# crstnbr/detqmc

Measured on AMD Instinct MI355X. Metric: DQMC sweeps/sec (SDW-O2 L=16 beta=10 fp64), higher is better.
Workload: dtype f64; 1 GPU; DetSDW O(2) L=16 beta=10 dtau=0.1 s=10 checkerboard delayed(32) sweepThermalization, 512 independent chains per GPU (1 process x 4 kernel contexts x 128 lockstep chains), stabilisation=qr; n_g=512, m=100, replicas_per_gpu=512, processes_per_gpu=1, contexts_per_process=4, chains_per_context=128, launch=self

## Files before the change

detqmc_amd/_lib.py:

```python
import ctypes as C
import os

HERE = os.path.dirname(os.path.abspath(__file__))
LIB_PATH = os.path.join(HERE, "lib", "libdetqmc_amd.so")


class DqmcError(RuntimeError):

    def __init__(self, code, msg):
        super().__init__(f"[dqmc {code}] {msg}")
        self.code = code


DQMC_TD_EVERY_SLICE = 0x100
DETSDW_TD_EVERY_SLICE = 0x100
DETSDW_TD_FINE_ON_DEVICE = 0x200
DETSDW_OBS_FINE = 0x100
DQMC_SERIES_AUTO_REBIN, DQMC_SERIES_TRACK_VARIANCE = 1, 2
DETSDW_SERIES_NO_HOST_COPY = 1
DETSDW_SERIES_PHI = 2
DETSDW_FM_EQ_CORRELATORS = 0x100
DQMC_TD_PH_BAND = 0x100
DETSDW_TD_PH_BAND = 0x100
DETSDW_FM_EQ_BAND = 0x200
DQMC_SERIES_MATS_BAND, DQMC_SERIES_EQ_BAND = 128, 256
DQMC_SERIES_MATS_CUSTOM, DQMC_SERIES_EQ_CUSTOM = 512, 1024
DQMC_SERIES_MATS_CUSTOM_PAIR, DQMC_SERIES_EQ_CUSTOM_PAIR = 2048, 4096
DQMC_SERIES_GREEN_MATRIX = 8192
DQMC_CUSTOM_MAX = 4
DETSDW_OBS_FAMILY_SLICE, DETSDW_OBS_FAMILY_EQ, DETSDW_OBS_FAMILY_TD, DETSDW_OBS_FAMILY_PHI = 0, 1, 2, 3
(DETSDW_OBS_KIND_SITE, DETSDW_OBS_KIND_TAU, DETSDW_OBS_KIND_TAU_Q0, DETSDW_OBS_KIND_ROW_SCALAR, DETSDW_OBS_KIND_CORR, DETSDW_OBS_KIND_SQ,
 DETSDW_OBS_KIND_GREEN_MATRIX, DETSDW_OBS_KIND_PHI_CHI, DETSDW_OBS_KIND_PHI_SCALARS) = range(9)


class dqmc_cplx(C.Structure):
    _fields_ = [("re", C.c_double), ("im", C.c_double)]


class dqmc_tuning(C.Structure):
    _fields_ = [("pipeline", C.c_int32), ("qr_variant", C.c_int32), ("green_variant", C.c_int32),
                ("max_jacobi_sweeps", C.c_int32), ("proposal_budget", C.c_int32), ("decide_threads", C.c_int32), ("bmult_path", C.c_int32)]


DQMC_TUNING_NO_RNG_LOOKAHEAD = 0x100


class dqmc_schedule_info(C.Structure):
    _fields_ = [("pipelined", C.c_int32), ("proposal_budget", C.c_int32), ("blocks_pipelined", C.c_uint64),
                ("blocks_sequential", C.c_uint64), ("qr_block_gram_schmidt", C.c_int32), ("green_lu", C.c_int32),
                ("cholqr_fallbacks", C.c_uint64), ("uniform_windows_advanced", C.c_uint64), ("uniform_windows_pushed", C.c_uint64)]


class dqmc_params(C.Structure):
    _fields_ = [("opdim", C.c_int32), ("L", C.c_int32), ("m", C.c_int32), ("s", C.c_int32),
                ("delaySteps", C.c_int32), ("bc", C.c_int32), ("weakZflux", C.c_int32),
                ("phi2bosons", C.c_int32), ("device", C.c_int32), ("stabilisation", C.c_int32),
                ("cb_none", C.c_int32), ("model", C.c_int32),
                ("dtau", C.c_double), ("r", C.c_double), ("c", C.c_double), ("u", C.c_double),
                ("lambda_", C.c_double),
                ("txhor", C.c_double), ("txver", C.c_double), ("tyhor", C.c_double), ("tyver", C.c_double),
                ("mux", C.c_double), ("muy", C.c_double), ("accRatio", C.c_double), ("cdwU", C.c_double),
                ("rng_window_per_site", C.c_int32), ("timedisplaced", C.c_int32),
                ("tuning", dqmc_tuning), ("td_particle_hole", C.c_int32)]


class dqmc_update_state(C.Structure):
    _fields_ = [("phiDelta", C.c_double), ("targetAccRatio", C.c_double), ("lastAccRatio", C.c_double),
                ("ra_runningAverage", C.c_double), ("ra_values", C.c_double * 100),
                ("ra_samplesAdded", C.c_int32), ("ra_head", C.c_int32),
                ("rng_consumed", C.c_uint64), ("rng_avail", C.c_uint64),
                ("error", C.c_int32), ("reserved", C.c_int32),
                ("angleDelta", C.c_double), ("scaleDelta", C.c_double),
                ("curminAngleDelta", C.c_double), ("curmaxAngleDelta", C.c_double),
                ("curminScaleDelta", C.c_double), ("curmaxScaleDelta", C.c_double),
                ("rot_runningAverage", C.c_double), ("rot_values", C.c_double * 100),
                ("scl_runningAverage", C.c_double), ("scl_values", C.c_double * 100),
                ("rot_samplesAdded", C.c_int32), ("rot_head", C.c_int32), ("scl_samplesAdded", C.c_int32), ("scl_head", C.c_int32)]


class dqmc_series_state(C.Structure):
    _fields_ = [("bin_size", C.c_int), ("max_bins", C.c_int), ("nfreq", C.c_int), ("parts", C.c_int), ("flags", C.c_int),
                ("bins_closed", C.c_int), ("sweeps_in_open_bin", C.c_int), ("nb", C.c_int),
                ("samples", C.c_longlong), ("rebins", C.c_longlong), ("sample_len", C.c_size_t)]


class dqmc_profile(C.Structure):
    _fields_ = [("ms", C.c_double * 8), ("launches", C.c_uint64 * 8),
                ("svd_calls", C.c_uint64), ("svd_sweeps_total", C.c_uint64), ("svd_sweeps_max", C.c_uint64),
                ("qr_calls", C.c_uint64), ("gemm_flops", C.c_double), ("decomp_round_ms", C.c_double),
                ("decomp_rounds", C.c_uint64), ("blocks_nonempty", C.c_uint64), ("chains", C.c_uint64),
                ("updates_accepted", C.c_uint64), ("lu_calls", C.c_uint64),
                ("sub_ms", C.c_double * 4), ("sub_launches", C.c_uint64 * 4), ("sub_flops", C.c_double * 4), ("sub_bytes", C.c_double * 4)]


class detsdw_params(C.Structure):
    _fields_ = [("opdim", C.c_int32), ("L", C.c_int32), ("m", C.c_int32), ("s", C.c_int32),
                ("delaySteps", C.c_int32), ("globalShift", C.c_int32), ("globalUpdateInterval", C.c_int32),
                ("weakZflux", C.c_int32), ("phi2bosons", C.c_int32), ("device", C.c_int32),
                ("simindex", C.c_int32), ("rngSeed", C.c_uint32), ("has_mux_muy", C.c_int32),
                ("updateMethod", C.c_int32), ("bc", C.c_char * 16),
                ("beta", C.c_double), ("dtau", C.c_double),
                ("r", C.c_double), ("c", C.c_double), ("u", C.c_double), ("lambda_", C.c_double),
                ("txhor", C.c_double), ("txver", C.c_double), ("tyhor", C.c_double), ("tyver", C.c_double),
                ("mu", C.c_double), ("mux", C.c_double), ("muy", C.c_double),
                ("accRatio", C.c_double), ("cdwU", C.c_double),
                ("stabilisation", C.c_int32), ("cb_none", C.c_int32),
                ("wolffClusterUpdate", C.c_int32), ("wolffClusterShiftUpdate", C.c_int32),
                ("repeatWolffPerSweep", C.c_int32), ("fermionMeasurements", C.c_int32),
                ("spinProposalMethod", C.c_int32), ("adaptScaleVariance", C.c_int32), ("repeatUpdateInSlice", C.c_int32),
                ("timeDisplacedMeasurements", C.c_int32),
                ("tuning", dqmc_tuning), ("timeDisplacedParticleHole", C.c_int32)]


class detsdw_info(C.Structure):
    _fields_ = [("opdim", C.c_int32), ("L", C.c_int32), ("N", C.c_int32), ("MSF", C.c_int32),
                ("n_g", C.c_int32), ("m", C.c_int32), ("s", C.c_int32), ("n", C.c_int32),
                ("performedSweeps", C.c_int32), ("lastSweepDir", C.c_int32),
                ("acceptedGlobalShifts", C.c_int32), ("attemptedGlobalShifts", C.c_int32),
                ("currentTimeslice", C.c_int32), ("reserved", C.c_int32),
                ("acceptedWolffClusterUpdates", C.c_int32), ("attemptedWolffClusterUpdates", C.c_int32),
                ("acceptedWolffClusterShiftUpdates", C.c_int32), ("attemptedWolffClusterShiftUpdates", C.c_int32),
                ("addedWolffClusterSize", C.c_double),
                ("beta", C.c_double), ("dtau", C.c_double),
                ("phiDelta", C.c_double), ("lastAccRatioLocal_phi", C.c_double), ("r", C.c_double),
                ("angleDelta", C.c_double), ("scaleDelta", C.c_double),
                ("rngDrawn", C.c_uint64)]


class detsdw_observable_desc(C.Structure):
    _fields_ = [(f, C.c_int32) for f in ("family", "block", "component", "kind", "fine", "has_fine_twin", "has_matsubara",
                                          "series_part", "series_bit")]


# ... 306 lines not shown
```

detqmc_amd/csrc/dqmc_context.hip:

```cpp
#include "dqmc_ctx.h"
#include <cmath>
#include <complex>
#include <cstddef>
#include <cstdio>
#include <cstdlib>
#include <cstring>
#include <string>
#include <vector>

void build_tournament(int nblk, std::vector<int>& out);

thread_local std::string g_err;

template<class T>
static int dalloc(dqmc_ctx* c, T** p, size_t count) {
    const size_t bytes = (count * sizeof(T) + 255) & ~(size_t)255;
    *p = (T*)(uintptr_t)(c->arena_off + 256);
    c->fixups.push_back((void**)p);
    c->arena_off += bytes;
    return 0;
}
static int arena_commit(dqmc_ctx* c) {
    const size_t cs = c->arena_off;
    void* q = nullptr;
// ... 229 lines not shown
    const double t = p.txhor, mu = p.mux;
    std::vector<hc> Em, Ep;
    if (p.cb_none) {
        std::vector<hc> T((size_t)N * N, hc(0.0));
        for (int i = 0; i < N; ++i) T[(size_t)i * N + i] = -mu;
        for (int site = 0; site < N; ++site)
            for (int dir = 0; dir < 4; ++dir) T[(size_t)neigh[dir * N + site] * N + site] -= t;
        herm_exp_dense(N, T, -p.dtau, +p.dtau, Em, Ep);
    } else {
        const double ch = std::cosh(p.dtau * t), sh = std::sinh(p.dtau * t);
        auto bond_matrix = [&](int dirn, int parity, double shv) {
            std::vector<double> M((size_t)N * N, 0.0);
            for (int i = 0; i < N; ++i) M[(size_t)i * N + i] = ch;
            for (int y = 0; y < L; ++y)
                for (int x = 0; x < L; ++x) {
                    const int coord = dirn == 0 ? x : y;
                    if ((coord & 1) != parity) continue;
                    const int a = y * L + x, b = neigh[(dirn == 0 ? 0 : 2) * N + a];
                    M[(size_t)a * N + b] += shv; M[(size_t)b * N + a] += shv;
                }
            return M;
        };
        auto mul = [&](const std::vector<double>& A, const std::vector<double>& B) {
            std::vector<double> C((size_t)N * N, 0.0);
            for (int i = 0; i < N; ++i) for (int k = 0; k < N; ++k) { const double a = A[(size_t)i * N + k]; if (a != 0.0) for (int j = 0; j < N; ++j) C[(size_t)i * N + j] += a * B[(size_t)k * N + j]; }
            return C;
        };
        const std::vector<double> F = mul(mul(bond_matrix(0, 0, sh), bond_matrix(0, 1, sh)), mul(bond_matrix(1, 0, sh), bond_matrix(1, 1, sh)));
        const std::vector<double> Fi = mul(mul(bond_matrix(1, 1, -sh), bond_matrix(1, 0, -sh)), mul(bond_matrix(0, 1, -sh), bond_matrix(0, 0, -sh)));
        Em.assign((size_t)N * N, hc(0.0)); Ep.assign((size_t)N * N, hc(0.0));
        for (size_t i = 0; i < (size_t)N * N; ++i) { Em[i] = F[i]; Ep[i] = Fi[i]; }
    }
    out_minus.assign((size_t)ng * ng, hc(0.0)); out_plus.assign((size_t)ng * ng, hc(0.0));
    for (int b = 0; b < 2; ++b)
        for (int i = 0; i < N; ++i) for (int j = 0; j < N; ++j) {
            out_minus[(size_t)(b * N + j) * ng + (b * N + i)] = Em[(size_t)i * N + j];
            out_plus[(size_t)(b * N + j) * ng + (b * N + i)] = Ep[(size_t)i * N + j];
        }
}

static int alloc_qr_work(dqmc_ctx* c) {
    const int ng = c->n_g, np = (ng + 15) / 16;
    const size_t n2 = (size_t)ng * ng;
    int rc;
#define A_(x) if ((rc = (x))) return rc;
    A_(dalloc(c, &c->qw.V, n2)); A_(dalloc(c, &c->qw.T, (size_t)np * 2 * 256));
    A_(dalloc(c, &c->qw.W, (size_t)16 * ng)); A_(dalloc(c, &c->qw.W2, (size_t)16 * ng)); A_(dalloc(c, &c->qw.Rneg, (size_t)32 * ng));
    if (ng > 1024) { c->qw.part_count = (size_t)ng * 64 * 8; A_(dalloc(c, &c->qw.part, c->qw.part_count)); }
    A_(dalloc(c, &c->qr_perm, (size_t)ng)); A_(dalloc(c, &c->lu_swaps, (size_t)LU_SWAP_INTS)); A_(dalloc(c, &c->lu_tneg, (size_t)ng * 32)); A_(dalloc(c, &c->qr_perm_inv, (size_t)ng)); A_(dalloc(c, &c->qr_dinv, (size_t)ng));
    A_(dalloc(c, &c->rmax_inv, (size_t)ng)); A_(dalloc(c, &c->rmin, (size_t)ng));
    A_(dalloc(c, &c->lmax_inv, (size_t)ng)); A_(dalloc(c, &c->lmin, (size_t)ng));
#undef A_
    return 0;
}

static int alloc_slot(dqmc_ctx* c, UdVSlot& sl) {
    size_t n2 = (size_t)c->n_g * c->n_g;
    int rc;
    if ((rc = dalloc(c, &sl.U, n2))) return rc;
    if ((rc = dalloc(c, &sl.d, (size_t)c->n_g))) return rc;
    if ((rc = dalloc(c, &sl.Vt, n2))) return rc;
    return 0;
}

extern "C" int dqmc_create(const dqmc_params* p, dqmc_ctx** out) { return dqmc_create_batch(p, 1, out); }
static int create_fill(dqmc_ctx* c, const dqmc_params* p);

extern "C" int dqmc_create_batch(const dqmc_params* p, int nchains, dqmc_ctx** out) {
    if (!p || !out) return fail(DQMC_EINVAL, "null argument");
    *out = nullptr;
    if (nchains < 1 || nchains > 1024) return fail(DQMC_EINVAL, "nchains must be in 1..1024");
    if (p->opdim < 1 || p->opdim > 3) return fail(DQMC_EINVAL, "opdim must be 1, 2 or 3");
    if (p->L < 2 || (p->L % 2) != 0)
        return fail(DQMC_EINVAL, "Checker board decomposition only supported for even linear lattice sizes");
    if (p->weakZflux && p->opdim != 2) return fail(DQMC_EINVAL, "Magnetic field currently only supported for opdim=2");
    if (p->m < 2 || p->s < 1 || p->s >= p->m) return fail(DQMC_EINVAL, "need 0 < s < m");
    const int N = p->L * p->L, MSF = p->opdim == 3 ? 4 : 2;
    if (p->delaySteps < 1 || p->delaySteps > N) return fail(DQMC_EINVAL, "delaySteps must be in 1..N");
    if (MSF * p->delaySteps > DQMC_MAX_WDIM) return fail(DQMC_EINVAL, "MSF*delaySteps must be <= 64 on this build");
    if (p->bc < 0 || p->bc > 3) return fail(DQMC_EINVAL, "bc");
    if (p->tuning.decide_threads != 0 && p->tuning.decide_threads != 256 && p->tuning.decide_threads != 512)
        return fail(DQMC_EINVAL, "tuning.decide_threads must be 0, 256 or 512");
    {
        const int path = p->tuning.bmult_path & ~DQMC_TUNING_NO_RNG_LOOKAHEAD;
        if (p->tuning.bmult_path < 0 || path > 2) return fail(DQMC_EINVAL, "tuning.bmult_path must be 0, 1 or 2");
    }
    if (p->stabilisation != DQMC_STAB_SVD && p->stabilisation != DQMC_STAB_QR) return fail(DQMC_EINVAL, "stabilisation");
    if (!(p->dtau > 0)) return fail(DQMC_EINVAL, "dtau");
    if (p->model != DQMC_MODEL_SDW && p->model != DQMC_MODEL_HUBBARD) return fail(DQMC_EINVAL, "model");
    if (p->model == DQMC_MODEL_HUBBARD) {
        if (p->opdim != 1 || p->weakZflux || p->bc != DQMC_BC_PBC || p->delaySteps != 1)
            return fail(DQMC_EINVAL, "Hubbard replica: opdim must be 1, delaySteps 1, bc pbc, no flux");
        if (!(p->u >= 0)) return fail(DQMC_EINVAL, "Hubbard replica: U must be >= 0 (alpha = acosh(e^{dtau U / 2}))");
        if (p->cdwU != 0.0) return fail(DQMC_EINVAL, "Hubbard replica: cdwU must be 0");
    }
    const int ng = MSF * N;
    if (p->stabilisation == DQMC_STAB_SVD && ng > 2304) return fail(DQMC_EINVAL, "n_g > 2304 not supported by the Jacobi kernel instantiations");
    if (ng > 4096) return fail(DQMC_EINVAL, "n_g > 4096 not supported by the QR panel kernel instantiations");

    int ndev = 0;
    if (hipGetDeviceCount(&ndev) != hipSuccess || ndev <= 0) return fail(DQMC_ENODEV, "no HIP device available");
    if (p->device < 0 || p->device >= ndev) return fail(DQMC_ENODEV, "device ordinal out of range");
    HIPCHK(hipSetDevice(p->device));

    dqmc_ctx* c = new dqmc_ctx();
    c->p = *p;
    c->nb = nchains;
    c->N = N; c->MSF = MSF; c->n_g = ng; c->m = p->m; c->s = p->s; c->D = p->delaySteps;
    c->n = (p->m + p->s - 1) / p->s;
    const int rc = create_fill(c, p);
    if (rc != DQMC_OK) { dqmc_destroy(c); return rc; }
    *out = c;
    return DQMC_OK;
}

static int create_fill(dqmc_ctx* c, const dqmc_params* p) {
    const int N = c->N, MSF = c->MSF, ng = c->n_g;
    HIPCHK(hipStreamCreateWithFlags(&c->st, hipStreamNonBlocking));
    HIPCHK(hipStreamCreateWithFlags(&c->st2, hipStreamNonBlocking));
    HIPCHK(hipEventCreateWithFlags(&c->ev_win, hipEventDisableTiming));
    HIPCHK(hipEventCreateWithFlags(&c->ev_flush, hipEventDisableTiming));
    HIPCHK(hipEventCreateWithFlags(&c->ev_tail, hipEventDisableTiming));
    HIPCHK(hipEventCreateWithFlags(&c->ev_adv, hipEventDisableTiming));

    DevModel& hm = c->hm;
    memset(&hm, 0, sizeof(hm));
    hm.opdim = p->opdim; hm.MSF = MSF; hm.L = p->L; hm.N = N; hm.ng = ng; hm.m = p->m; hm.s = p->s; hm.n = c->n;
    hm.D = p->delaySteps; hm.P = N / 4; hm.phi2bosons = p->phi2bosons;
    hm.pbudget = p->delaySteps >= 8 ? 2 * p->delaySteps : 0;
    if (p->tuning.proposal_budget != 0) hm.pbudget = p->tuning.proposal_budget < 0 ? 0 : p->tuning.proposal_budget;
    if (hm.pbudget > 0 && hm.pbudget < p->delaySteps) hm.pbudget = p->delaySteps;
    hm.decide_nt = p->tuning.decide_threads;
    hm.bmult_path = p->tuning.bmult_path & ~DQMC_TUNING_NO_RNG_LOOKAHEAD;
#ifdef DQMC_DECIDE_TIMING
    hm.dbg = (getenv("DQMC_DECIDE_TIMING") && atoi(getenv("DQMC_DECIDE_TIMING"))) ? 8 : 0;
#endif
    hm.dtau = p->dtau; hm.r = p->r; hm.c = p->c; hm.u = p->u; hm.lambda = p->lambda;
    hm.ov[0] = std::exp(p->dtau * p->mux); hm.ov[1] = std::exp(p->dtau * p->muy);
    hm.ovinv[0] = std::exp(-p->dtau * p->mux); hm.ovinv[1] = std::exp(-p->dtau * p->muy);

    std::vector<int> psites, neigh;
    std::vector<hc> pmats;
    std::vector<double> pabcd;
    build_tables(*p, psites, pmats, pabcd, neigh);
    std::vector<hc> pmats_h;
    std::vector<double> pabcd_h;
    { std::vector<int> ps2, nb2; build_tables(*p, ps2, pmats_h, pabcd_h, nb2, true); }
    int *d_psites, *d_neigh; cplx *d_pmats, *d_pmats_h; double *d_pabcd, *d_pabcd_h;
    int rc;
#define A_(x) if ((rc = (x))) return rc;
    A_(salloc(c, &d_psites, psites.size()));
    A_(salloc(c, &d_neigh, neigh.size()));
    A_(salloc(c, &d_pmats, pmats.size()));
    A_(salloc(c, &d_pabcd, pabcd.size()));
    HIPCHK(copy_sync(c, d_pabcd, pabcd.data(), pabcd.size() * sizeof(double), hipMemcpyHostToDevice));
    HIPCHK(copy_sync(c, d_psites, psites.data(), psites.size() * sizeof(int), hipMemcpyHostToDevice));
    HIPCHK(copy_sync(c, d_neigh, neigh.data(), neigh.size() * sizeof(int), hipMemcpyHostToDevice));
    HIPCHK(copy_sync(c, d_pmats, pmats.data(), pmats.size() * sizeof(hc), hipMemcpyHostToDevice));
    A_(salloc(c, &d_pmats_h, pmats_h.size()));
    A_(salloc(c, &d_pabcd_h, pabcd_h.size()));
    HIPCHK(copy_sync(c, d_pmats_h, pmats_h.data(), pmats_h.size() * sizeof(hc), hipMemcpyHostToDevice));
    HIPCHK(copy_sync(c, d_pabcd_h, pabcd_h.data(), pabcd_h.size() * sizeof(double), hipMemcpyHostToDevice));
    hm.psites = d_psites; hm.neigh = d_neigh; hm.pmats = d_pmats; hm.pabcd = d_pabcd; hm.pm_real = p->weakZflux ? 0 : 1;
    hm.pmats_h = d_pmats_h; hm.pabcd_h = d_pabcd_h;
    if (p->model == DQMC_MODEL_HUBBARD) {
        hm.hubbard = 1; hm.dense = 1;
        hm.ov[0] = hm.ov[1] = hm.ovinv[0] = hm.ovinv[1] = 1.0;
        const double alpha = std::acosh(std::exp(p->dtau * p->u * 0.5));
        hm.hub_exp_alpha[0] = std::exp(alpha); hm.hub_exp_alpha[1] = std::exp(-alpha);
        c->hub_e_m2a = std::exp(-2.0 * alpha * 1.0); c->hub_e_p2a = std::exp(2.0 * alpha * 1.0);
        std::vector<hc> em, ep;
        build_hubbard_propK(*p, neigh, em, ep);
        const size_t nn = (size_t)ng * ng;
        A_(salloc(c, &c->propK[0], nn)); A_(salloc(c, &c->propK[1], nn)); A_(dalloc(c, &c->Tdense, nn));
        HIPCHK(copy_sync(c, c->propK[0], em.data(), nn * sizeof(hc), hipMemcpyHostToDevice));
        HIPCHK(copy_sync(c, c->propK[1], ep.data(), nn * sizeof(hc), hipMemcpyHostToDevice));
    } else if (p->cb_none) {
        hm.dense = 1;
        hm.ov[0] = hm.ov[1] = hm.ovinv[0] = hm.ovinv[1] = 1.0;
        std::vector<hc> em, ep;
        build_dense_propK(*p, neigh, MSF, em, ep);
        const size_t nn = (size_t)ng * ng;
        A_(salloc(c, &c->propK[0], nn)); A_(salloc(c, &c->propK[1], nn)); A_(dalloc(c, &c->Tdense, nn));
        HIPCHK(copy_sync(c, c->propK[0], em.data(), nn * sizeof(hc), hipMemcpyHostToDevice));
        HIPCHK(copy_sync(c, c->propK[1], ep.data(), nn * sizeof(hc), hipMemcpyHostToDevice));
        build_dense_propK(*p, neigh, MSF, em, ep, 0.5);
        A_(salloc(c, &c->propKh[0], nn)); A_(salloc(c, &c->propKh[1], nn));
        HIPCHK(copy_sync(c, c->propKh[0], em.data(), nn * sizeof(hc), hipMemcpyHostToDevice));
        HIPCHK(copy_sync(c, c->propKh[1], ep.data(), nn * sizeof(hc), hipMemcpyHostToDevice));
    }

    const size_t nphi = (size_t)(p->m + 1) * p->opdim * N, ncs = (size_t)(p->m + 1) * N;
    A_(dalloc(c, &c->phi, nphi)); A_(dalloc(c, &c->coshT, ncs)); A_(dalloc(c, &c->sinhT, ncs));
    A_(dalloc(c, &c->phi_bak, nphi)); A_(dalloc(c, &c->cosh_bak, ncs)); A_(dalloc(c, &c->sinh_bak, ncs));
    if (p->cdwU != 0.0) { A_(dalloc(c, &c->cdwl, ncs)); A_(dalloc(c, &c->cdwC, ncs)); A_(dalloc(c, &c->cdwS, ncs)); }

    const size_t n2 = (size_t)ng * ng;
    A_(dalloc(c, &c->G, n2)); A_(dalloc(c, &c->G_bak, n2));
    A_(dalloc(c, &c->sv, (size_t)ng)); A_(dalloc(c, &c->sv_bak, (size_t)ng));
    c->storage.resize(c->n + 1); c->storage_bak.resize(c->n + 1);
    for (int l = 0; l <= c->n; ++l) { A_(alloc_slot(c, c->storage[l])); A_(alloc_slot(c, c->storage_bak[l])); }
    A_(alloc_slot(c, c->spare)); A_(alloc_slot(c, c->tmpudv));
    A_(dalloc(c, &c->T1, n2)); A_(dalloc(c, &c->T2, n2)); A_(dalloc(c, &c->T3, n2)); A_(dalloc(c, &c->T4, n2));
    A_(dalloc(c, &c->sw.A, n2)); A_(dalloc(c, &c->sw.V, n2));
    A_(dalloc(c, &c->sw.norms, (size_t)ng)); A_(dalloc(c, &c->sw.rnorms, (size_t)ng)); A_(dalloc(c, &c->sw.flagT, 1)); A_(dalloc(c, &c->sw.rank, (size_t)ng));
    A_(salloc(c, &c->sw.flag, 1));
    HIPCHK(hipHostMalloc((void**)&c->sw.hflag, 2 * sizeof(unsigned long long), hipHostMallocMapped));
    c->sw.hflag[0] = 0; c->sw.hflag[1] = 0;
    HIPCHK(hipHostGetDevicePointer((void**)&c->sw.hslot_dev, c->sw.hflag, 0));
    A_(salloc(c, &c->sw.seqctr, 1));
    HIPCHK(hipMemsetAsync(c->sw.seqctr, 0, sizeof(unsigned long long), c->st));
    c->sw.host_seq = &c->jacobi_host_seq;
    c->sw.last_residual = &c->last_svd_residual;
    c->sw.sweep_graph = &c->jacobi_graph;
    {
        int bw = svd_block_cols(ng);
        int nblk = ng / bw;
        std::vector<int> rounds;
        build_tournament(nblk, rounds);
        int* d_rounds;
        A_(salloc(c, &d_rounds, rounds.size()));
        HIPCHK(copy_sync(c, d_rounds, rounds.data(), rounds.size() * sizeof(int), hipMemcpyHostToDevice));
        c->sw.rounds = d_rounds; c->sw.nrounds = nblk - 1; c->sw.nblk = nblk;
    }
    c->stab = p->stabilisation;
    if (p->tuning.max_jacobi_sweeps > 0) c->max_jacobi_sweeps = p->tuning.max_jacobi_sweeps;
    c->qr_bgs = p->tuning.qr_variant == 2 || (p->tuning.qr_variant == 0 && ng > 1024);
    c->green_lu = ng <= 512 && p->tuning.green_variant != 1;
    if (c->stab == DQMC_STAB_QR) A_(alloc_qr_work(c));
    A_(alloc_slot(c, c->eye));
    const int WD = MSF * c->D;
    const int WD8 = (WD + 7) & ~7;
    A_(dalloc(c, &c->X, (size_t)ng * WD8)); A_(dalloc(c, &c->Gr, (size_t)WD8 * ng)); A_(dalloc(c, &c->W, (size_t)WD * WD));
    {
        const int want = p->tuning.pipeline;
        const bool on = want > 0 || (want == 0 && ng > 1024 && c->nb >= 2);
        if (on && p->model == DQMC_MODEL_SDW && hm.pbudget > 0 && MSF * hm.pbudget <= 512) {
            c->pipelined = true;
            c->pipe_P = hm.pbudget;
            A_(dalloc(c, &c->Gwin, (size_t)MSF * hm.pbudget * (MSF * hm.pbudget + 1)));
        }
    }
    if (p->rng_window_per_site < 0 || p->rng_window_per_site > 4096) return fail(DQMC_EINVAL, "rng_window_per_site");
    c->uni_cap = (size_t)(p->rng_window_per_site > 0 ? p->rng_window_per_site : (p->opdim + 1 + (p->cdwU != 0.0 ? 2 : 0))) * N * p->m + 64;
    A_(dalloc(c, &c->uniforms, c->uni_cap));
    if (!(p->tuning.bmult_path & DQMC_TUNING_NO_RNG_LOOKAHEAD)) {
        A_(dalloc(c, &c->uniforms_next, c->uni_cap)); A_(dalloc(c, &c->uni_tail, c->uni_cap));
    }
    A_(dalloc(c, &c->us, 1));
    A_(dalloc(c, &c->scalar_out, 8));
    A_(salloc(c, &c->shift_buf, (size_t)c->nb * 3));
    auto acc_alloc = [c](int id, size_t count) { c->acc[id].n = count; return dalloc(c, &c->acc[id].p, count); };
    A_(acc_alloc(ACC_SLICE, measure_accum_doubles(N, p->L)));
    const int td_level = p->timedisplaced & ~DQMC_TD_EVERY_SLICE;
    if (p->timedisplaced < 0 || td_level > 2) return fail(DQMC_EINVAL, "timedisplaced must be 0, 1 or 2 (| DQMC_TD_EVERY_SLICE)");
    if ((p->timedisplaced & DQMC_TD_EVERY_SLICE) && !td_level) return fail(DQMC_EINVAL, "DQMC_TD_EVERY_SLICE needs timedisplaced >= 1");
    if (p->model == DQMC_MODEL_HUBBARD && (p->timedisplaced || p->td_particle_hole)) {
        if (p->timedisplaced != 1 || p->td_particle_hole != 1)
            return fail(DQMC_EINVAL, "Hubbard replica: timedisplaced = 1 with td_particle_hole = 1 is the only time-displaced reservation (every "
                                     "other value of the two fields: SDW model only)");
        c->td_reserved = true;
        A_(dalloc(c, &c->GT0, n2)); A_(dalloc(c, &c->G0T, n2)); A_(dalloc(c, &c->td_W, n2));
        if (c->stab != DQMC_STAB_QR) { A_(alloc_qr_work(c)); A_(dalloc(c, &c->td_sv, (size_t)ng)); }
        A_(dalloc(c, &c->G00, n2)); A_(dalloc(c, &c->ph_H, n2));
        A_(acc_alloc(ACC_HUB_TD, hubbard_td_doubles(N, c->n)));
    } else if (td_level) {
        if (p->model != DQMC_MODEL_SDW) return fail(DQMC_EINVAL, "timedisplaced: SDW model only");
        c->td_reserved = true;
        A_(dalloc(c, &c->GT0, n2)); A_(dalloc(c, &c->G0T, n2)); A_(dalloc(c, &c->td_W, n2));
        if (c->stab != DQMC_STAB_QR) { A_(alloc_qr_work(c)); A_(dalloc(c, &c->td_sv, (size_t)ng)); }
        A_(acc_alloc(ACC_TD, measure_td_doubles(p->L, c->n)));
        if (td_level == 2) A_(acc_alloc(ACC_TD_PAIR, measure_td_pair_doubles(N, c->n)));
    }
    const int ph_level = p->td_particle_hole & ~DQMC_TD_PH_BAND;
    const bool ph_band = p->td_particle_hole >= 0 && (p->td_particle_hole & DQMC_TD_PH_BAND);
    if (p->td_particle_hole < 0 || ph_level > 2) return fail(DQMC_EINVAL, "td_particle_hole must be 0, 1 or 2 (| DQMC_TD_PH_BAND)");
    if (ph_band && !ph_level) return fail(DQMC_EINVAL, "DQMC_TD_PH_BAND needs td_particle_hole >= 1");
    if (ph_level && p->model == DQMC_MODEL_SDW) {
        if (!td_level) return fail(DQMC_EINVAL, "td_particle_hole needs timedisplaced >= 1");
        A_(dalloc(c, &c->G00, n2)); A_(dalloc(c, &c->ph_H, n2));
        A_(dalloc(c, &c->ph_ob, measure_td_ph_onebody_cplx(N)));
        A_(acc_alloc(ACC_TD_PH, measure_td_ph_doubles(N, c->n)));
    }
    if (ph_level == 2) {
        std::vector<hc> bt;
        build_bond_table(*p, neigh, MSF, bt);
        A_(salloc(c, &c->cur_bt, bt.size()));
        HIPCHK(copy_sync(c, c->cur_bt, bt.data(), bt.size() * sizeof(hc), hipMemcpyHostToDevice));
        A_(dalloc(c, &c->cur_ob, measure_td_current_onebody_cplx(N)));
        A_(acc_alloc(ACC_TD_CUR, measure_td_current_doubles(N, c->n)));
    }
    if (p->timedisplaced & DQMC_TD_EVERY_SLICE) {
        c->td_fine = true;
        A_(dalloc(c, &c->fGT0, n2)); A_(dalloc(c, &c->fG0T, n2)); A_(dalloc(c, &c->fGTT, n2));
        const bool on[4] = {true, td_level == 2, ph_level >= 1, ph_level == 2};
        for (int ch = 0; ch < 4; ++ch)
            if (on[ch]) A_(acc_alloc(ACC_FINE0 + ch, (size_t)(p->m + 1) * (1 + measure_td_row_doubles(ch, N, p->L))));
    }
    if (ph_band) {
        A_(dalloc(c, &c->band_ob, measure_td_band_onebody_cplx(N)));
        A_(acc_alloc(ACC_TD_BAND, measure_td_band_doubles(N, c->n)));
        if (c->td_fine) A_(acc_alloc(ACC_FINE0 + 4, (size_t)(p->m + 1) * (1 + measure_td_row_doubles(4, N, p->L))));
    }
    A_(arena_commit(c));
#undef A_
    for (int id = 0; id < ACC_EQ; ++id) c->acc[id].stride = c->lc.cs;
    c->acc[ACC_HUB_TD].stride = c->lc.cs;
    c->qw.err = &c->us->chol_fail;
    hm.phi = c->phi; hm.coshT = c->coshT; hm.sinhT = c->sinhT;
    if (p->cdwU != 0.0) {
        hm.cdw_on = 1; hm.cdwl = c->cdwl; hm.cdwC = c->cdwC; hm.cdwS = c->cdwS;
// ... 237 lines not shown
    bool bgs = c->qr_bgs;
    if (bgs) {
        launches += run_qr_bgs(c->lc, n, c->sw.A, Qdst, c->qw);
        int failed = 0;
        { int rc = chol_failed(c, &failed); if (rc) return rc; }
        if (failed) {
            c->cholqr_fallbacks += 1;
            bgs = false;
            qr_reset_workspace(c->lc, n, c->qw);
            launch_udt_init(c->lc, M, n, cs, rs, c->qr_perm, transpose, c->sw.A, n);
            launches += 3;
        }
    }
    if (!bgs) launches += run_qr(c->lc, n, c->sw.A, form_q ? Qdst : nullptr, c->qw);
    c->qr_calls += 1;
    *out = QrOutcome{launches, bgs || form_q};
    return DQMC_OK;
}

static int udt_dev(dqmc_ctx* c, const cplx* M, const double* colscale, const double* rowscale, int kind, UdVSlot out, int lazy = 0) {
    const int n = c->n_g;
    const int transpose = (kind == KIND_L);
    ProfScope ps(c, FAM_JACOBI, 0);
    cplx* Q = transpose ? out.Vt : out.U;
    cplx* Tt = transpose ? out.U : out.Vt;
    QrOutcome qr;
    { int rc = qr_factorise(c, M, colscale, rowscale, transpose, Q, true, &qr); if (rc) return rc; }
    launch_udt_diag(c->lc, c->sw.A, n, out.d);
    if (lazy) launch_udt_lazy(c->lc, out.d, c->qr_perm, n, c->qr_dinv, c->qr_perm_inv);
    else launch_udt_tmat(c->lc, c->sw.A, out.d, c->qr_perm, n, Tt);
    c->fam_launches[FAM_JACOBI] += qr.launches + 2;
    return DQMC_OK;
}

enum ZRoute { Z_LU, Z_QR_REFLECTORS, Z_QR_EXPLICIT };
struct ZFactors {
    ZRoute route;
    const cplx* tri;
    const cplx* Q;
    int adjoint;
};
static int factorise_z(dqmc_ctx* c, double* svout, ZFactors* z, int* launches) {
    const int n = c->n_g;
    ProfScope ps(c, FAM_JACOBI, 0);
    if (c->green_lu) {
        *launches = run_lu(c->lc, n, c->T2, c->qr_perm, c->lu_swaps, c->lu_tneg);
        c->lu_calls += 1;
        *z = ZFactors{Z_LU, c->T2, nullptr, 1};
    } else {
        QrOutcome qr;
        { int rc = qr_factorise(c, c->T2, nullptr, nullptr, 0, c->T4, false, &qr); if (rc) return rc; }
        *launches = qr.launches;
        *z = ZFactors{qr.q_explicit ? Z_QR_EXPLICIT : Z_QR_REFLECTORS, c->sw.A, qr.q_explicit ? c->T4 : nullptr, 0};
    }
    launch_logdet_vector(c->lc, z->tri, c->rmax_inv, c->lmax_inv, n, svout);
    *launches += 1;
    return DQMC_OK;
}
static int left_half(dqmc_ctx* c, const ZFactors& z, const cplx* X, const double* scale, cplx* dst) {
    ProfScope ps(c, FAM_JACOBI, 0);
    if (z.route == Z_LU) {
        const ColSrc src = {X, c->n_g, nullptr, scale};
        return run_trsm_right_upper(c->lc, c->n_g, z.tri, dst, c->qw, 0, 0, &src);
    }
    launch_permute_scale_cols(c->lc, X, scale, c->qr_perm, c->n_g, dst);
    return 1 + run_trsm_right_upper(c->lc, c->n_g, z.tri, dst, c->qw);
}
static int right_half(dqmc_ctx* c, const ZFactors& z, const cplx* Yh, const double* scale, cplx* dst, cplx* stage) {
    const int n = c->n_g;
    int launches = 1;
    {
        ProfScope ps(c, FAM_JACOBI, 0);
        if (z.route == Z_LU) {
            const ColSrc src = {Yh, n, c->qr_perm, scale};
            launches = run_trsm_right_upper(c->lc, n, z.tri, dst, c->qw, 1, 1, &src);
        } else if (z.route == Z_QR_REFLECTORS) {
            launch_udt_init(c->lc, Yh, n, scale, nullptr, nullptr, 1, dst, n);
            launches += run_qr_apply_q(c->lc, n, dst, c->qw, 1);
        } else launch_udt_init(c->lc, Yh, n, scale, nullptr, nullptr, 1, stage, n);
    }
    if (z.route == Z_QR_EXPLICIT) run_gemm(c, gemm_square(c, z.Q, 1, stage, 0, dst));
    return launches;
}

static int green_qr(dqmc_ctx* c, const UdVSlot* Lp, const UdVSlot* Rp, cplx* Gout, double* svout, bool td = false) {
    const UdVSlot& L = Lp ? *Lp : c->eye;
    const UdVSlot& R = Rp ? *Rp : c->eye;
    {
        ProfScope ps(c, FAM_OTHER, 2);
        launch_split_scales(c->lc, R.d, c->n_g, c->rmax_inv, c->rmin);
        launch_split_scales(c->lc, L.d, c->n_g, c->lmax_inv, c->lmin);
    }
    GemmArgs g = gemm_square(c, R.U, 1, L.Vt, 0, c->T2);
    g.rowscale = c->rmax_inv; g.colscale = c->lmax_inv;
    run_gemm(c, g);
    g = gemm_square(c, R.Vt, 1, L.U, 0, c->T2);
    g.rowscale = c->rmin; g.colscale = c->lmin; g.accumulate = 1;
    run_gemm(c, g);
    ZFactors z;
    int launches = 0;
    { int rc = factorise_z(c, svout, &z, &launches); if (rc) return rc; }
    launches += left_half(c, z, L.Vt, c->lmax_inv, c->T3);
    launches += right_half(c, z, R.U, c->rmax_inv, c->T1, c->sw.V);
    if (Gout) run_gemm(c, gemm_square(c, c->T3, 0, c->T1, z.adjoint, Gout));
    if (td) {
        cplx* Bmin = z.route == Z_LU ? c->T4 : c->T2;
        launches += right_half(c, z, R.Vt, c->rmin, Bmin, c->td_W);
        launches += left_half(c, z, L.U, c->lmin, c->td_W);
        run_gemm(c, gemm_square(c, c->T3, 0, Bmin, z.adjoint, c->GT0));
        g = gemm_square(c, c->td_W, 0, c->T1, z.adjoint, c->G0T);
        g.negate = 1;
        run_gemm(c, g);
        if (c->G00) {
            g = gemm_square(c, c->td_W, 0, Bmin, z.adjoint, c->G00);
            g.negate = 1;
            run_gemm(c, g);
            ProfScope ps(c, FAM_OTHER, 1);
            launch_add_diag(c->lc, c->G00, c->eye.d, c->n_g);
        }
    }
    c->fam_launches[FAM_JACOBI] += launches;
    return DQMC_OK;
}

static int udv_dev(dqmc_ctx* c, const cplx* M, const double* colscale, const double* rowscale, UdVSlot out);
static int decompose(dqmc_ctx* c, const cplx* M, const double* colscale, const double* rowscale, int kind, UdVSlot out) {
    if (c->stab == DQMC_STAB_QR) return udt_dev(c, M, colscale, rowscale, kind, out);
    return udv_dev(c, M, colscale, rowscale, out);
}

static int decompose_chained(dqmc_ctx* c, const cplx* M, const double* colscale, const double* rowscale, int kind, UdVSlot out,
                             const cplx* Aold) {
    cplx* dest = (kind == KIND_R) ? out.Vt : out.U;
    if (c->stab == DQMC_STAB_QR) {
        int rc = udt_dev(c, M, colscale, rowscale, kind, out, 1);
        if (rc) return rc;
        GemmArgs g = gemm_square(c, Aold, 0, c->sw.A, 1, dest);
        g.a_kgather = c->qr_perm_inv; g.b_lower = 1; g.colscale = c->qr_dinv;
        run_gemm(c, g);
        return DQMC_OK;
    }
    UdVSlot t = out;
    if (kind == KIND_R) t.Vt = c->tmpudv.Vt; else t.U = c->tmpudv.U;
    int rc = decompose(c, M, colscale, rowscale, kind, t);
    if (rc) return rc;
    run_gemm(c, gemm_square(c, Aold, 0, (kind == KIND_R) ? c->tmpudv.Vt : c->tmpudv.U, 0, dest));
    return DQMC_OK;
}

static void green_from_svd(dqmc_ctx* c, const cplx* Vl, const cplx* Ur, const UdVSlot& t) {
    run_gemm(c, gemm_square(c, Vl, 0, t.Vt, 0, c->T3));
    run_gemm(c, gemm_square(c, Ur, 0, t.U, 0, c->T4));
    GemmArgs g = gemm_square(c, c->T3, 0, c->T4, 1, c->G);
    g.kscale = c->sv; g.kscale_invert = 1;
    run_gemm(c, g);
}
static int green_from_udv(dqmc_ctx* c, const UdVSlot& L, const UdVSlot& R) {
    if (c->stab == DQMC_STAB_QR) return green_qr(c, &L, &R, c->G, c->sv, c->td_on);
    run_gemm(c, gemm_square(c, R.U, 1, L.Vt, 0, c->T2));
    GemmArgs g = gemm_square(c, R.Vt, 1, L.U, 0, c->T2);
    g.rowscale = R.d; g.colscale = L.d; g.accumulate = 1;
    run_gemm(c, g);
    UdVSlot t = c->tmpudv; t.d = c->sv;
    int rc = udv_dev(c, c->T2, nullptr, nullptr, t);
    if (rc) return rc;
    green_from_svd(c, L.Vt, R.U, t);
    if (c->td_on) return green_qr(c, &L, &R, nullptr, c->td_sv, true);
    return DQMC_OK;
}
static int green_from_eye(dqmc_ctx* c, const UdVSlot& R, int kind) {
    if (c->stab == DQMC_STAB_QR) return (kind == KIND_R) ? green_qr(c, nullptr, &R, c->G, c->sv) : green_qr(c, &R, nullptr, c->G, c->sv);
    run_gemm(c, gemm_square(c, R.U, 1, R.Vt, 0, c->T2));
    { ProfScope ps(c, FAM_OTHER, 1); launch_add_diag(c->lc, c->T2, R.d, c->n_g); }
    UdVSlot t = c->tmpudv; t.d = c->sv;
    int rc = udv_dev(c, c->T2, nullptr, nullptr, t);
    if (rc) return rc;
    green_from_svd(c, R.Vt, R.U, t);
    return DQMC_OK;
}

static int set_slot_identity(dqmc_ctx* c, UdVSlot& sl) {
    ProfScope ps(c, FAM_OTHER, 2);
    launch_set_identity(c->lc, sl.U, c->n_g);
    launch_set_identity(c->lc, sl.Vt, c->n_g);
    std::vector<double> ones(c->n_g, 1.0);
    for (int b = 0; b < c->nb; ++b)
        HIPCHK(hipMemcpyAsync(chainp(c, sl.d, b), ones.data(), c->n_g * sizeof(double), hipMemcpyHostToDevice, c->st));
    HIPCHK(hipStreamSynchronize(c->st));
    return DQMC_OK;
}

// ... 295 lines not shown
    const int adapt_what = adapt | (adapt_scale_variance ? 4 : 0);
    if (c->hm.hubbard) {
        ProfScope ps(c, FAM_UPDATE, 1);
        launch_hubbard_slice(c->lc, c->hm, c->us, c->uniforms, c->G, k, c->hub_e_m2a, c->hub_e_p2a);
        return finish(c, "dqmc_update_slice");
    }
    const int rounds = (c->N + c->D - 1) / c->D;
    const int WD = c->MSF * c->D;
    const bool pipe = c->pipelined;
    Launch lc2 = c->lc; lc2.st = c->st2;
    auto pass = [&](int cdw_pass, int thermal, int reset_nd, bool skip) -> int {
        const int* done = skip ? &c->us->slice_done : nullptr;
        for (int r = 0; r < rounds; ++r) {
            {
                ProfScope ps(c, FAM_UPDATE, 1);
                launch_update_decide(c->lc, nullptr, c->hm, c->us, c->uniforms, c->G, c->W, k, r == 0, cdw_pass ? 0 : thermal, cdw_pass,
                                     c->Gwin, (pipe && r > 0) ? c->pipe_P : 0, proposal, adapt_what, reset_nd && r == 0);
            }
            if (pipe && r > 0) HIPCHK(hipStreamWaitEvent(c->st, c->ev_flush, 0));
            {
                ProfScope ps(c, FAM_GATHER, 1);
                launch_update_gather(c->lc, c->hm, c->us, c->G, c->W, c->X, c->Gr, skip);
            }
            if (pipe) {
                { ProfScope ps(c, FAM_OTHER, 1); launch_update_window(c->lc, c->hm, c->us, c->G, c->X, c->Gr, c->Gwin, c->pipe_P); }
                HIPCHK(hipEventRecord(c->ev_win, c->st));
                HIPCHK(hipStreamWaitEvent(c->st2, c->ev_win, 0));
                {
                    ProfScope ps(c, FAM_FLUSH, 1, c->st2);
                    launch_flush(lc2, c->X, c->Gr, c->n_g, c->G, c->n_g, c->n_g, WD, &c->us->flush_k, 1);
                }
                HIPCHK(hipEventRecord(c->ev_flush, c->st2));
                c->blocks_pipelined += 1;
            } else {
                ProfScope ps(c, FAM_FLUSH, 1);
                launch_flush(c->lc, c->X, c->Gr, c->n_g, c->G, c->n_g, c->n_g, WD, &c->us->block_j, c->MSF, 0, done);
                c->blocks_sequential += 1;
            }
        }
        if (pipe) HIPCHK(hipStreamWaitEvent(c->st, c->ev_flush, 0));
        return DQMC_OK;
    };
    const bool skip = skip_final && !pipe;
    for (int rep = 0; rep < repeat; ++rep) {
        int rc = pass(0, (thermalization && rep == repeat - 1) ? 1 : 0, rep == 0, skip && rep == repeat - 1 && !c->hm.cdw_on);
        if (rc) return rc;
    }
    if (c->hm.cdw_on) { int rc = pass(1, 0, 0, skip); if (rc) return rc; }
    return finish(c, "dqmc_update_slice");
}

extern "C" int dqmc_update_slice_ex(dqmc_ctx* c, int k, int thermalization, int proposal, int adapt, int adapt_scale_variance, int repeat) {
    if (!c) return fail(DQMC_EINVAL, "null ctx");
    (void)hipSetDevice(c->p.device);
    return update_slice_run(c, k, thermalization, proposal, adapt, adapt_scale_variance, repeat, false);
}

extern "C" int dqmc_update_slice_final(dqmc_ctx* c, int k, int thermalization, int proposal, int adapt, int adapt_scale_variance, int repeat,
                                       int then_wrap_dir) {
    if (!c) return fail(DQMC_EINVAL, "null ctx");
    (void)hipSetDevice(c->p.device);
    if (then_wrap_dir != 0 && then_wrap_dir != DQMC_DOWN) return fail(DQMC_EINVAL, "updateInSlice: then_wrap_dir must be 0 or DQMC_DOWN");
    const bool skip = !c->pipelined && !c->hm.hubbard;
    int rc = update_slice_run(c, k, thermalization, proposal, adapt, adapt_scale_variance, repeat, skip);
    if (rc) return rc;
    if (!skip) return then_wrap_dir == DQMC_DOWN ? dqmc_wrap(c, DQMC_DOWN, k) : DQMC_OK;
    if (then_wrap_dir == DQMC_DOWN) c->currentTimeslice = k - 1;
    c->g_stale = true;
    return DQMC_OK;
}

extern "C" int dqmc_get_schedule_info(dqmc_ctx* c, dqmc_schedule_info* out) {
    if (!c || !out) return fail(DQMC_EINVAL, "null argument");
    memset(out, 0, sizeof(*out));
    out->pipelined = c->pipelined ? 1 : 0;
    out->proposal_budget = c->hm.pbudget;
    out->blocks_pipelined = c->blocks_pipelined;
    out->blocks_sequential = c->blocks_sequential;
    out->qr_block_gram_schmidt = (c->stab == DQMC_STAB_QR && c->qr_bgs) ? 1 : 0;
    out->green_lu = (c->stab == DQMC_STAB_QR && c->green_lu) ? 1 : 0;
    out->cholqr_fallbacks = c->cholqr_fallbacks;
    out->uniform_windows_advanced = c->windows_advanced;
    out->uniform_windows_pushed = c->windows_pushed;
    return DQMC_OK;
}

extern "C" int dqmc_get_update_state_host(dqmc_ctx* c, dqmc_update_state* out) {
    if (!c || !out) return fail(DQMC_EINVAL, "null argument");
    (void)hipSetDevice(c->p.device);
    HIPCHK(hipStreamSynchronize(c->st));
#ifdef DQMC_DECIDE_TIMING
    if (c->hm.dbg & 8) {
        DevUpdateState h;
        HIPCHK(copy_sync(c, &h, selp(c, c->us), sizeof(h), hipMemcpyDeviceToHost));
        fprintf(stderr, "[decide cycles, chain %d, %llu launches]", c->sel, h.dbg_cycles[12]);
        for (int i = 0; i < 10; ++i) fprintf(stderr, " t%d=%llu", i, h.dbg_cycles[i]);
        fprintf(stderr, "\n");
    }
#endif
    HIPCHK(copy_sync(c, out, &selp(c, c->us)->pub, sizeof(*out), hipMemcpyDeviceToHost));
    if (out->error) return fail(out->error, "device ran out of pre-drawn uniforms");
    return DQMC_OK;
}
extern "C" int dqmc_set_update_state_host(dqmc_ctx* c, const dqmc_update_state* in) {
    if (!c || !in) return fail(DQMC_EINVAL, "null argument");
    (void)hipSetDevice(c->p.device);
    HIPCHK(hipStreamSynchronize(c->st));
    HIPCHK(copy_sync(c, &selp(c, c->us)->pub, in, sizeof(*in), hipMemcpyHostToDevice));
    return DQMC_OK;
}

extern "C" int dqmc_bmult_host(dqmc_ctx* c, int side, int inverse, int k2, int k1, dqmc_cplx* A) {
    if (!c || !A) return fail(DQMC_EINVAL, "null argument");
    (void)hipSetDevice(c->p.device);
    if (!(k2 > k1) || k2 > c->m || k1 < 0) return fail(DQMC_EINVAL, "need 0 <= k1 < k2 <= m");
    const size_t n2 = (size_t)c->n_g * c->n_g;
    for (int b = 0; b < c->nb; ++b)
        HIPCHK(hipMemcpyAsync(chainp(c, c->T1, b), A, n2 * sizeof(cplx), hipMemcpyHostToDevice, c->st));
    bmult_dev(c, side, inverse, k2, k1, c->T1);
    HIPCHK(hipMemcpyAsync(A, selp(c, c->T1), n2 * sizeof(cplx), hipMemcpyDeviceToHost, c->st));
    HIPCHK(hipStreamSynchronize(c->st));
    return finish(c, "dqmc_bmult_host");
}
extern "C" int dqmc_bmult_src_host(dqmc_ctx* c, int side, int inverse, int k2, int k1, const dqmc_cplx* src, dqmc_cplx* out, dqmc_cplx* src_after) {
    if (!c || !src || !out) return fail(DQMC_EINVAL, "null argument");
    (void)hipSetDevice(c->p.device);
    if (!(k2 > k1) || k2 > c->m || k1 < 0) return fail(DQMC_EINVAL, "need 0 <= k1 < k2 <= m");
    const size_t n2 = (size_t)c->n_g * c->n_g;
    for (int b = 0; b < c->nb; ++b) {
        HIPCHK(hipMemcpyAsync(chainp(c, c->T3, b), src, n2 * sizeof(cplx), hipMemcpyHostToDevice, c->st));
        HIPCHK(hipMemsetAsync(chainp(c, c->T1, b), 0xff, n2 * sizeof(cplx), c->st));
    }
    bmult_dev(c, side, inverse, k2, k1, c->T1, c->T3);
    HIPCHK(hipMemcpyAsync(out, selp(c, c->T1), n2 * sizeof(cplx), hipMemcpyDeviceToHost, c->st));
    if (src_after) HIPCHK(hipMemcpyAsync(src_after, selp(c, c->T3), n2 * sizeof(cplx), hipMemcpyDeviceToHost, c->st));
    HIPCHK(hipStreamSynchronize(c->st));
    return finish(c, "dqmc_bmult_src_host");
}

extern "C" int dqmc_udv_decompose_host(dqmc_ctx* c, const dqmc_cplx* M, dqmc_cplx* U, double* d, dqmc_cplx* V_t,
                                       int* sweeps_used) {
    if (!c || !M || !U || !d || !V_t) return fail(DQMC_EINVAL, "null argument");
    (void)hipSetDevice(c->p.device);
    const size_t n2 = (size_t)c->n_g * c->n_g;
    for (int b = 0; b < c->nb; ++b)
        HIPCHK(hipMemcpyAsync(chainp(c, c->T1, b), M, n2 * sizeof(cplx), hipMemcpyHostToDevice, c->st));
    int rc = decompose(c, c->T1, nullptr, nullptr, KIND_R, c->tmpudv);
    if (rc) return rc;
    HIPCHK(hipStreamSynchronize(c->st));
    HIPCHK(copy_sync(c, U, selp(c, c->tmpudv.U), n2 * sizeof(cplx), hipMemcpyDeviceToHost));
    HIPCHK(copy_sync(c, d, selp(c, c->tmpudv.d), c->n_g * sizeof(double), hipMemcpyDeviceToHost));
    HIPCHK(copy_sync(c, V_t, selp(c, c->tmpudv.Vt), n2 * sizeof(cplx), hipMemcpyDeviceToHost));
    if (sweeps_used) *sweeps_used = c->last_svd_sweeps;
    return DQMC_OK;
}

static void stab_test_invalidate(dqmc_ctx* c) {
    c->g_stale = true;
    c->currentTimeslice = -1;
    c->td_slice = -1;
}
template<class T>
static int stab_upload(dqmc_ctx* c, T* dev, const void* host, size_t count) {
    for (int b = 0; b < c->nb; ++b)
        HIPCHK(hipMemcpyAsync(chainp(c, dev, b), (const T*)host + (size_t)b * count, count * sizeof(T), hipMemcpyHostToDevice, c->st));
    return DQMC_OK;
// ... 284 lines not shown
```

detqmc_amd/csrc/dqmc_ctx.h:

```cpp
#pragma once
#include "dqmc_internal.h"
#include <cstdint>
#include <cstdlib>
#include <string>
#include <utility>
#include <vector>

#define DQMC_PRIVATE __attribute__((visibility("hidden")))

extern DQMC_PRIVATE thread_local std::string g_err;
static int fail(int code, const std::string& msg) { g_err = msg; return code; }
#define HIPCHK(x)                                                                                       \
    do {                                                                                                \
        hipError_t e_ = (x);                                                                            \
        if (e_ != hipSuccess)                                                                           \
            return fail(DQMC_EHIP, std::string(#x) + ": " + hipGetErrorString(e_) + " (" + __FILE__ + ":" + \
                                       std::to_string(__LINE__) + ")");                                  \
    } while (0)

static bool sync_check_on() {
    static const bool on = getenv("DQMC_SYNC_CHECK") && atoi(getenv("DQMC_SYNC_CHECK")) != 0;
    return on;
}

struct UdVSlot { cplx* U; double* d; cplx* Vt; };

enum { FAM_BMULT = DQMC_FAM_BMULT, FAM_GEMM = DQMC_FAM_GEMM, FAM_JACOBI = DQMC_FAM_DECOMP, FAM_UPDATE = DQMC_FAM_DECIDE,
       FAM_OTHER = DQMC_FAM_OTHER, FAM_GATHER = DQMC_FAM_GATHER, FAM_FLUSH = DQMC_FAM_FLUSH, FAM_ROUNDS = 7, FAM_COUNT = DQMC_FAM_COUNT };

enum { TD_CHANNELS = 8 };
enum { ACC_SLICE, ACC_TD, ACC_TD_PAIR, ACC_TD_PH, ACC_TD_CUR, ACC_TD_BAND, ACC_TD_CUSTOM, ACC_TD_CUSTOM_PAIR, ACC_TD_GREEN_MATRIX, ACC_FINE0,
       ACC_EQ = ACC_FINE0 + TD_CHANNELS, ACC_EQ_BAND, ACC_EQ_CUSTOM, ACC_EQ_CUSTOM_PAIR, ACC_HUB_EQ, ACC_HUB_TD, ACC_COUNT };
struct AccBlock { double* p; size_t n, stride; const char* missing; };

struct dqmc_ctx {
    dqmc_params p;
    DevModel hm;
    hipStream_t st = nullptr;
    hipStream_t st2 = nullptr;
    hipEvent_t ev_win = nullptr, ev_flush = nullptr;
    cplx* Gwin = nullptr;
    int pipe_P = 0;
    bool pipelined = false;
    uint64_t blocks_pipelined = 0, blocks_sequential = 0, cholqr_fallbacks = 0;
    bool qr_bgs = false, green_lu = false;
    std::vector<int> err_host;
    Launch lc{nullptr, 1, 0};
    int nb = 1, sel = 0;
    char* arena = nullptr;
    size_t arena_off = 0;
    std::vector<void**> fixups;
    int n_g = 0, MSF = 0, N = 0, m = 0, s = 0, n = 0, D = 0;
    std::vector<void*> allocs;
    double *phi = nullptr, *coshT = nullptr, *sinhT = nullptr;
    double *cdwl = nullptr, *cdwC = nullptr, *cdwS = nullptr;
    double *phi_bak = nullptr, *cosh_bak = nullptr, *sinh_bak = nullptr;
    cplx *G = nullptr, *G_bak = nullptr;
    double *sv = nullptr, *sv_bak = nullptr;
    std::vector<UdVSlot> storage, storage_bak;
    UdVSlot spare{}, tmpudv{};
    cplx *T1 = nullptr, *T2 = nullptr, *T3 = nullptr, *T4 = nullptr;
    cplx *propK[2] = {nullptr, nullptr}, *Tdense = nullptr;
    cplx *propKh[2] = {nullptr, nullptr};
    AccBlock acc[ACC_COUNT] = {
        {nullptr, 0, 0, "the context has no measurement accumulators"},
        {nullptr, 0, 0, "context created without dqmc_params::timedisplaced"},
        {nullptr, 0, 0, "context created without dqmc_params::timedisplaced == 2"},
        {nullptr, 0, 0, "context created without dqmc_params::td_particle_hole"},
        {nullptr, 0, 0, "context created without dqmc_params::td_particle_hole = 2"},
        {nullptr, 0, 0, "context created without DQMC_TD_PH_BAND"},
        {nullptr, 0, 0, "no user-defined bilinear is set (dqmc_set_custom_bilinears), or the context was created without dqmc_params::td_particle_hole"},
        {nullptr, 0, 0, "no user-defined pair operator is set (dqmc_set_custom_pair_operators), or the context was created without dqmc_params::timedisplaced"},
        {nullptr, 0, 0, "the averaged Green's function block is switched off (dqmc_set_green_matrix)"},
        {nullptr, 0, 0, "no every-slice block for this channel"}, {nullptr, 0, 0, "no every-slice block for this channel"},
        {nullptr, 0, 0, "no every-slice block for this channel"}, {nullptr, 0, 0, "no every-slice block for this channel"},
        {nullptr, 0, 0, "no every-slice block for this channel"}, {nullptr, 0, 0, "no every-slice block for this channel"},
        {nullptr, 0, 0, "no every-slice block for this channel"}, {nullptr, 0, 0, "no every-slice block for this channel"},
        {nullptr, 0, 0, "the equal-time correlators have never been enabled (dqmc_set_equal_time_correlators)"},
        {nullptr, 0, 0, "the equal-time band correlators have never been enabled (dqmc_set_equal_time_band)"},
        {nullptr, 0, 0, "no user-defined bilinear is set (dqmc_set_custom_bilinears)"},
        {nullptr, 0, 0, "no user-defined pair operator is set (dqmc_set_custom_pair_operators)"},
        {nullptr, 0, 0, "the Hubbard equal-time correlators have never been enabled (dqmc_hubbard_set_equal_time_correlators)"},
        {nullptr, 0, 0, "Hubbard context created without dqmc_params::timedisplaced = 1 and td_particle_hole = 1"}};
    bool td_reserved = false, td_on = false;
    int td_slice = -1;
    cplx *GT0 = nullptr, *G0T = nullptr, *td_W = nullptr;
    double* td_sv = nullptr;
    cplx *G00 = nullptr, *ph_H = nullptr, *ph_ob = nullptr;
    cplx *cur_bt = nullptr, *cur_ob = nullptr;
    cplx *band_ob = nullptr;
    bool td_fine = false;
    int fine_slice = -1;
    cplx *fGT0 = nullptr, *fG0T = nullptr, *fGTT = nullptr;
    double* mats_out = nullptr;
    size_t mats_cap = 0;
    bool eq_on = false;
    cplx* eq_ob = nullptr;
    bool hub_eq_on = false;
    double* hub_eq_sc = nullptr;
    bool eqb_on = false;
    cplx* eqb_ob = nullptr;
    int cst_count = 0;
    cplx cst_M[DQMC_CUSTOM_MAX * 16] = {}, cst_M2[DQMC_CUSTOM_MAX * 16] = {};
    unsigned cst_mask[DQMC_CUSTOM_MAX] = {}, cst_mask2[DQMC_CUSTOM_MAX] = {};
    bool eqc_on = false;
    cplx *cst_td_ob = nullptr, *cst_eq_ob = nullptr;
    cplx cst_Mx[DQMC_CUSTOM_MAX * 16] = {}, cst_My[DQMC_CUSTOM_MAX * 16] = {};
    bool cst_bond_on = false;
    CustomBond cst_bond = {};
    int cpr_count = 0;
    cplx cpr_F0[DQMC_CUSTOM_MAX * 16] = {}, cpr_Fx[DQMC_CUSTOM_MAX * 16] = {}, cpr_Fy[DQMC_CUSTOM_MAX * 16] = {}, cpr_Fa[DQMC_CUSTOM_MAX * 16] = {};
    unsigned cpr_mask[DQMC_CUSTOM_MAX] = {};
    bool eqp_on = false, cpr_bond_on = false;
    CustomPair cpr_bond = {};
    bool gm_on = false;
    struct Series {
        bool open = false, formed = false;
        int bin_size = 0, max_bins = 0, nfreq = 0, parts = 0, closed = 0, in_open = 0;
        int flags = 0;
        long long samples = 0, rebins = 0;
        size_t S = 0, off[14] = {}, len[14] = {};
        double *sample = nullptr, *openbin = nullptr, *bins = nullptr, *bad = nullptr, *trig = nullptr, *stat = nullptr;
        double *var = nullptr;
        double *binning = nullptr;
        size_t binning_cap = 0;
        double *vertex = nullptr;
        size_t vertex_cap = 0;
        void *vertex_tab = nullptr;
// ... 135 lines not shown
```

detqmc_amd/csrc/dqmc_internal.h:

```cpp
#pragma once
#include <hip/hip_runtime.h>
#include <stdint.h>
#include "../../include/dqmc_hip.h"

#include <stdlib.h>
#include <float.h>
static inline const char* dev_knob(const char* name) {
#ifdef DQMC_DEV_KNOBS
    return getenv(name);
#else
    (void)name;
    return nullptr;
#endif
}

typedef double2 cplx;

#define DQMC_MAX_MSF 4
#define DQMC_MAX_WDIM 64
#define DQMC_DECIDE_WIDE_MAX_CHAINS 32

enum { SUBFAM_LU_UPDATE = 0, SUBFAM_FACT_GEMM = 1, SUBFAM_COUNT = 4 };
struct SubProf { void (*begin)(void* user, int sub); void (*end)(void* user, int sub, double flops, double bytes); void* user; };
struct Launch { hipStream_t st; int nb; size_t cs; const SubProf* sub = nullptr; };
// ... 48 lines not shown
    const cplx* pmats;
    const double* pabcd;
    int pm_real;
    const cplx* pmats_h;
    const double* pabcd_h;
    double* phi;
    double* coshT;
    double* sinhT;
    int cdw_on;
    double* cdwl;
    double* cdwC;
    double* cdwS;
    double cdw_cosh[2], cdw_sinh[2];
    double cdw_gamma[2];
    const int* neigh;
    int hubbard;
    double hub_exp_alpha[2];
};
__device__ __forceinline__ DevModel chain_model(DevModel dm, size_t cs) {
    dm.phi = chain_ptr(dm.phi, cs); dm.coshT = chain_ptr(dm.coshT, cs); dm.sinhT = chain_ptr(dm.sinhT, cs);
    if (dm.cdw_on) { dm.cdwl = chain_ptr(dm.cdwl, cs); dm.cdwC = chain_ptr(dm.cdwC, cs); dm.cdwS = chain_ptr(dm.cdwS, cs); }
    return dm;
}

struct DevUpdateState {
    dqmc_update_state pub;
    int site_cursor;
    int acc_count;
    int block_j;
    int slice_done;
    int flush_k;
    int nd_has;
    double nd_cached;
    int chol_fail;
    double r;
    int block_sites[DQMC_MAX_WDIM];
    unsigned long long blocks_nonempty;
    unsigned long long updates_accepted;
    unsigned long long dbg_cycles[16];
};

void launch_bmult(const Launch& lc, const DevModel* dm, const DevModel& hm, int side, int inverse,
                  int kfirst, int kstep, int kcount, cplx* A, int lda, int shift = 0,
                  const cplx* Asrc = nullptr);

struct ColSrc { const cplx* X; int ld; const int* idx; const double* scale; };
static inline ColSrc col_src_from(const ColSrc& s, int j0) {
    ColSrc r = s;
    if (!r.X) return r;
    if (r.idx) r.idx += j0;
    else { r.X += (size_t)j0 * r.ld; if (r.scale) r.scale += j0; }
    return r;
}
#ifdef __HIPCC__
__device__ __forceinline__ cplx col_src_value(cplx v, double s) {
#pragma clang fp contract(off)
    return make_double2(v.x * s, v.y * s);
}
#endif

struct GemmArgs {
    const cplx* A; int lda; int opA;
    const cplx* B; int ldb; int opB;
    cplx* C; int ldc;
    int M, N, K;
    const int* Kdev;
    int Kmul;
    const double* kscale;
    int kscale_invert;
    const double* rowscale;
    const double* colscale;
    int accumulate;
    int negate;
    int sharedA, sharedB;
    const int* a_kgather;
    int b_lower;
    int ksplit; cplx* part;
    size_t part_count;
    int tag;
    ColSrc csrc;
};
void launch_gemm(const Launch& lc, const GemmArgs& a);
int launch_gemm_path(const Launch& lc, const GemmArgs& a, int path);
struct GemmPlan { int tile, ksplit, xcd; };
GemmPlan gemm_plan(const GemmArgs& a, int nb);
void launch_flush(const Launch& lc, const cplx* X, const cplx* GrT, int ld, cplx* G, int ldc, int n, int Kmax,
                  const int* Kdev, int Kmul, int tag = 0,
                  const int* skip = nullptr);

struct SvdWork {
    cplx* A; cplx* V; double* norms; double* rnorms; int* rank; int* flagT;
    unsigned long long* flag; double* last_residual;
    unsigned long long* hflag;
    unsigned long long* hslot_dev;
    unsigned long long* seqctr;
    unsigned long long* host_seq;
    const int* rounds; int nrounds; int nblk;
    hipGraphExec_t* sweep_graph;
};
struct SvdProfHooks { void (*begin)(void* user); void (*end)(void* user, int launches); void* user; };
int run_svd(const Launch& lc, int n, const cplx* M, int ldm, const double* colscale, const double* rowscale,
            cplx* U, double* d, cplx* Vt, const SvdWork& w, int max_sweeps, const SvdProfHooks* hooks = nullptr);
int svd_block_cols(int n);

__device__ __forceinline__ void cdw_site_terms(const DevModel& dm, size_t idx, double sign, double c, double& c0, double& c1, double& xs) {
    if (dm.cdw_on) {
        const double cC = dm.cdwC[idx], sC = dm.cdwS[idx];
        c0 = c * cC - sign * sC; c1 = c * cC + sign * sC; xs *= cC;
    } else { c0 = c; c1 = c; }
}
void launch_cdw_terms(const Launch& lc, const DevModel& hm);
void launch_update_decide(const Launch& lc, const DevModel* dm, const DevModel& hm, DevUpdateState* us,
                          const double* uniforms, const cplx* G, cplx* W, int k, int first, int thermal, int cdw_pass = 0,
                          const cplx* Gwin = nullptr, int winP = 0,
                          int proposal = 0, int adapt_what = 0, int reset_nd = 0);
void launch_update_window(const Launch& lc, const DevModel& hm, DevUpdateState* us, const cplx* G, const cplx* X, const cplx* GrT,
                          cplx* Gw, int P);
void launch_update_gather(const Launch& lc, const DevModel& hm, const DevUpdateState* us, const cplx* G,
                          const cplx* W, cplx* X, cplx* GrT, int skip_done = 0);
void launch_advance_uniforms(const Launch& lc, DevUpdateState* us, const double* cur, const double* tail, double* nw,
                             const unsigned long long* off, size_t need);

void launch_hubbard_vscale(const Launch& lc, const DevModel& hm, int side, int inverse, int k, cplx* A, int lda);
void launch_hubbard_slice(const Launch& lc, const DevModel& hm, DevUpdateState* us, const double* uniforms, cplx* G, int k,
                          double e_m2a, double e_p2a);
void launch_hubbard_measure(const Launch& lc, const DevModel& hm, const cplx* G, double* acc);
#define HUB_EQ_CH 8
#define HUB_TD_CH 6
size_t hubbard_corr_scratch_doubles(int N);
size_t hubbard_eq_doubles(int N);
size_t hubbard_td_doubles(int N, int n);
void launch_hubbard_corr_prep(const Launch& lc, const DevModel& hm, const cplx* T, const cplx* S, const cplx* Gt, const cplx* G0, double* sc,
                              size_t scs);
void launch_hubbard_eq_corr(const Launch& lc, const DevModel& hm, const cplx* G, const double* sc, size_t scs, double* acc, size_t acs);
void launch_hubbard_td_corr(const Launch& lc, const DevModel& hm, const cplx* GT0, const double* sc, size_t scs, double* acc, size_t acs,
                            int row, int rows);

void launch_cosh_sinh(const Launch& lc, const DevModel& hm);
void launch_set_identity(const Launch& lc, cplx* A, int n);
void launch_conj_transpose(const Launch& lc, const cplx* A, cplx* B, int n);
void launch_add_diag(const Launch& lc, cplx* A, const double* d, int n);
void launch_copy(const Launch& lc, const cplx* A, cplx* B, size_t count);
void launch_copy_bytes(const Launch& lc, const void* src, void* dst, size_t bytes);
void launch_phi_sq_sum(const Launch& lc, const DevModel& hm, double* out);
void launch_gather_scalars(const Launch& lc, const double* src, double factor, double* dst);
void launch_phi_action(const Launch& lc, const DevModel& hm, const DevUpdateState* us, double* out);
void launch_phi_shift(const Launch& lc, const DevModel& hm, const double* shifts );
void launch_measure_accum(const Launch& lc, const DevModel& hm, const cplx* gs, double* acc);
size_t measure_accum_doubles(int N, int L);
void launch_measure_td(const Launch& lc, const DevModel& hm, const cplx* gs, double* acc, int row, int rows);
size_t measure_td_row_doubles(int channel, int N, int L);
void launch_td_ends(const Launch& lc, const cplx* G, cplx* a_t0, cplx* a_0t, cplx* b_t0, cplx* b_0t, cplx* gtt, int ng);
size_t measure_td_doubles(int L, int n);
bool launch_td_matsubara(const Launch& lc, const DevModel& hm, const double* acc, int channel, int nfreq, int apbx, int apby,
                         double* out, double* bad, size_t out_chain_stride = 0, int custom_count = 0, size_t custom_chain_bytes = 0);
bool td_matsubara_fits(const DevModel& hm, int channel, int nfreq);
bool launch_series_eq_sample(const Launch& lc, const DevModel& hm, const double* eqacc, size_t eq_n, int nch, const double* trig, double* sample,
                             size_t S, size_t off, double* bad);
void launch_series_band_derived(const Launch& lc, const DevModel& hm, const double* bins, size_t S, int B, size_t off, double* value, double* err);
void launch_series_custom_derived(const Launch& lc, const DevModel& hm, const double* bins, size_t S, int B, size_t off, int count, int qx, int qy,
                                  double* value, double* err);
size_t series_eq_sample_lds_bytes(int L);
void launch_series_accum(const Launch& lc, const double* sample, double* open, double* closed, size_t n, int close, int bin_size);
void launch_series_accum_routed(const Launch& lc, const double* const* src, double* open, double* closed, size_t S, int close, int bin_size);
void launch_series_stats(const Launch& lc, const double* bins, size_t n, int B, double* mean, double* err);
void launch_series_derived(const Launch& lc, const DevModel& hm, const double* bins, size_t S, int B, int nfreq, long long off_eq,
                           long long off_cur, double* value, double* err);
bool launch_series_phi_sample(const Launch& lc, const DevModel& hm, const double* trig, const double* ttab, int nfreq, double* sample,
                              size_t S, size_t off);
int series_phi_sample_fgroup(int L, int m, int nfreq);
hipError_t series_phi_sample_prepare();
void launch_series_phi_derived(const Launch& lc, const DevModel& hm, const double* bins, size_t S, int B, int nfreq, size_t off,
                               double* value, double* err);
void launch_series_rebin(const Launch& lc, double* bins, size_t n, int half);
void launch_series_welford(const Launch& lc, const double* sample, const double* const* src, double* w, double* m2, size_t S, long long cnt);
void launch_series_binning(const Launch& lc, const double* bins, const double* m2, size_t n, int B, int levels, int bin_size,
                           long long samples, double* err, double* tau);
void launch_measure_td_pair(const Launch& lc, const DevModel& hm, const cplx* gs, double* acc, int row, int rows);
size_t measure_td_pair_doubles(int N, int n);
void launch_td_ph_onebody(const Launch& lc, const DevModel& hm, const cplx* gs, cplx* ob, int t);
void launch_measure_td_ph(const Launch& lc, const DevModel& hm, const cplx* gs, const cplx* hs, const cplx* ob, double* acc, int row, int rows);
size_t measure_td_ph_doubles(int N, int n);
size_t measure_td_ph_onebody_cplx(int N);
void launch_measure_eq_corr(const Launch& lc, const DevModel& hm, const cplx* gs, cplx* ob, double* acc);
size_t measure_eq_doubles(int N);
size_t measure_eq_onebody_cplx(int N);
void launch_td_current_onebody(const Launch& lc, const DevModel& hm, const cplx* gs, const cplx* bt, cplx* ob, int t);
void launch_measure_td_current(const Launch& lc, const DevModel& hm, const cplx* gs, const cplx* hs, const cplx* bt, const cplx* ob, double* acc, int row, int rows);
size_t measure_td_current_doubles(int N, int n);
size_t measure_td_current_onebody_cplx(int N);
size_t measure_td_current_bond_cplx(int N, int opdim);
void launch_td_band_onebody(const Launch& lc, const DevModel& hm, const cplx* gs, cplx* ob, int t);
void launch_measure_td_band(const Launch& lc, const DevModel& hm, const cplx* gs, const cplx* hs, const cplx* ob, double* acc, int row, int rows);
size_t measure_td_band_doubles(int N, int n);
size_t measure_td_band_onebody_cplx(int N);
void launch_measure_eq_band(const Launch& lc, const DevModel& hm, const cplx* gs, cplx* ob, double* acc);
size_t measure_eq_band_doubles(int N);
size_t measure_eq_band_onebody_cplx(int N);
struct CustomBond { const cplx* tab; const unsigned* mk; unsigned parts[DQMC_CUSTOM_MAX]; };
size_t measure_custom_bond_table_cplx(int count, int N);
void launch_td_custom_onebody(const Launch& lc, const DevModel& hm, int count, const cplx* M, const unsigned* mask, const cplx* gs, cplx* ob, int t,
                              const CustomBond* bond = nullptr);
void launch_measure_td_custom(const Launch& lc, const DevModel& hm, int count, const cplx* M, const unsigned* mask, const cplx* gs, const cplx* hs,
                              const cplx* ob, double* acc, size_t acs, int row, int rows, const CustomBond* bond = nullptr);
void launch_measure_eq_custom(const Launch& lc, const DevModel& hm, int count, const cplx* M, const unsigned* mask, const cplx* M2, const unsigned* mask2,
                              const cplx* gs, cplx* ob, double* acc, const CustomBond* bond = nullptr);
struct CustomPair { const cplx* tab; const unsigned* mk; unsigned parts[DQMC_CUSTOM_MAX]; };
size_t measure_custom_pair_table_cplx(int count, int N);
void launch_measure_custom_pair(const Launch& lc, const DevModel& hm, int count, const cplx* Fa, const unsigned* mask, const cplx* gs, double* acc,
                                size_t acs, int row, int rows, const CustomPair* pair = nullptr);
size_t measure_green_matrix_row_doubles(int opdim, int N);
void launch_measure_green_matrix(const Launch& lc, const DevModel& hm, const cplx* gs, double* acc, size_t acs, int row, int rows, int apbx, int apby);
void launch_series_green_sample(const Launch& lc, const DevModel& hm, const double* fine, size_t chain_bytes, double* sample, size_t S, size_t off,
                                double* bad);
size_t series_pair_bubble_lds_bytes(int opdim, int N);
bool launch_series_pair_vertex(const Launch& lc, const DevModel& hm, const double* bins, const double* mean, const double* trig, size_t S, int B,
                               int nfreq, size_t off_chi, size_t off_g, int count, const CustomPair& pair, int qx, int qy, int apbx, int apby,
                               double* pb, double* value, double* err);
size_t series_ph_bubble_lds_bytes(int opdim, int N);
bool launch_series_ph_vertex(const Launch& lc, const DevModel& hm, const double* bins, const double* mean, const double* trig, size_t S, int B,
                             int nfreq, size_t off_chi, size_t off_g, int count, const CustomBond& bond, int qx, int qy, int apbx, int apby,
                             double* pb, double* value, double* err);
struct GreenCheckFold { double* table; size_t table_stride; int row; const double* d; const double* sv; };
size_t green_diff_partial_doubles(int n);
void launch_green_keep(const Launch& lc, const cplx* G, cplx* keep, size_t keep_stride, size_t count);
void launch_green_diff(const Launch& lc, const cplx* Gw, size_t gw_stride, const cplx* Gf, int n, int ld, int N, double* part,
                       size_t part_stride, double* out, size_t out_stride, const GreenCheckFold* fold = nullptr);
size_t measure_custom_row_doubles(int count, int N);
size_t measure_td_custom_onebody_cplx(int count, int N);
size_t measure_eq_custom_onebody_cplx(int count, int N);

struct SvdProfHooks;
struct QrWork { cplx* V; cplx* T; cplx* W; cplx* W2; cplx* Rneg; const SvdProfHooks* apply_hooks; cplx* part; size_t part_count; int* err; };
int run_qr(const Launch& lc, int n, cplx* A, cplx* Q, const QrWork& w);
int run_qr_apply_q(const Launch& lc, int n, cplx* C, const QrWork& w, int trans);
int run_qr_bgs(const Launch& lc, int n, cplx* A, cplx* Q, const QrWork& w);
void qr_reset_workspace(const Launch& lc, int n, const QrWork& w);
int run_trsm_right_upper(const Launch& lc, int n, const cplx* R, cplx* C, const QrWork& w, int trans = 0, int unit = 0,
                         const ColSrc* src = nullptr);
#define LU_SWAP_INTS 128
int run_lu(const Launch& lc, int n, cplx* A, int* perm, int* swaps, cplx* tneg);
void launch_gather_scale_cols(const Launch& lc, const cplx* X, const double* cs, const int* perm, int n, cplx* Y);
void launch_udt_init(const Launch& lc, const cplx* M, int ldm, const double* cs, const double* rs, const int* perm,
                     int transpose, cplx* W, int n);
void launch_udt_diag(const Launch& lc, const cplx* R, int n, double* d);
void launch_udt_lazy(const Launch& lc, const double* d, const int* perm, int n, double* dinv, int* perm_inv);
void launch_udt_tmat(const Launch& lc, const cplx* R, const double* d, const int* perm, int n, cplx* Tt);
void launch_permute_scale_cols(const Launch& lc, const cplx* X, const double* cs, const int* perm, int n, cplx* Y);
void launch_split_scales(const Launch& lc, const double* d, int n, double* dmax_inv, double* dmin);
void launch_logdet_vector(const Launch& lc, const cplx* R, const double* a, const double* b, int n, double* sv);
void launch_scaled_norms_rank(const Launch& lc, const cplx* M, int ldm, const double* cs, const double* rs, int transpose,
                              int n, double* norms, int* rank, double* scratch_d);
```

detqmc_amd/csrc/kernels_gemm.hip:

```cpp
#include "dqmc_internal.h"
#include <mutex>
#include <algorithm>
#include <cstdlib>

typedef double v4d __attribute__((ext_vector_type(4)));

template<int TM, int TN, bool M3, int TAG, bool OPA, bool OPB, int FULL>
__global__ __launch_bounds__(256, 2) void k_zgemm(GemmArgs g, size_t cs, int nb) {
    constexpr int BM = 32 * TM, BN = 32 * TN, BK = 16;
    constexpr int NA = BM * BK / 256, NB_ = BN * BK / 256;
    __shared__ cplx sA[2][BK][BM + 1];
    __shared__ cplx sB[2][BK][BN + 1];
    const int tm = (g.M + BM - 1) / BM, tnn = (g.N + BN - 1) / BN;
    int chain, tile;
    xcd_chain_tile(tm * tnn, nb, chain, tile);
    if (!g.sharedA) g.A = chain_ptr_i(g.A, cs, chain);
    if (!g.sharedB) g.B = chain_ptr_i(g.B, cs, chain);
    g.C = chain_ptr_i(g.C, cs, chain);
    if constexpr (!FULL) { g.Kdev = chain_ptr_i(g.Kdev, cs, chain); g.kscale = chain_ptr_i(g.kscale, cs, chain); }
    g.rowscale = chain_ptr_i(g.rowscale, cs, chain); g.colscale = chain_ptr_i(g.colscale, cs, chain);
    g.a_kgather = chain_ptr_i(g.a_kgather, cs, chain);
    g.csrc.X = chain_ptr_i(g.csrc.X, cs, chain); g.csrc.idx = chain_ptr_i(g.csrc.idx, cs, chain); g.csrc.scale = chain_ptr_i(g.csrc.scale, cs, chain);

    int K = g.K;
    if (!FULL && g.Kdev) { int kd = (*g.Kdev) * g.Kmul; K = kd < K ? kd : K; }
    if (!FULL && K <= 0 && g.accumulate) return;
    int kslice0 = 0;
    if (!FULL && g.ksplit > 1) {
        const int kc = ((K + g.ksplit - 1) / g.ksplit + 15) & ~15;
        kslice0 = blockIdx.y * kc;
        K = min(K, kslice0 + kc);
        g.part = chain_ptr_i(g.part, cs, chain);
    }

    const int tid = threadIdx.x, lane = tid & 63, wave = tid >> 6;
    const int wm = wave >> 1, wn = wave & 1;
    const int i0 = (tile % tm) * BM, j0 = (tile / tm) * BN;
    const int l15 = lane & 15, l4 = lane >> 4;

    v4d acc_re[TM][TN], acc_im[TM][TN], acc_p2[M3 ? TM : 1][M3 ? TN : 1];
#pragma unroll
    for (int a = 0; a < TM; ++a)
#pragma unroll
        for (int b = 0; b < TN; ++b) { acc_re[a][b] = (v4d)(0.0); acc_im[a][b] = (v4d)(0.0); if (M3) acc_p2[a][b] = (v4d)(0.0); }

    auto mfma_tile = [&](int buf) {
#pragma unroll
        for (int kk = 0; kk < BK; kk += 4) {
            cplx af[TM], bf[TN];
#pragma unroll
            for (int a = 0; a < TM; ++a) af[a] = sA[buf][kk + l4][wm * 16 * TM + a * 16 + l15];
#pragma unroll
            for (int b = 0; b < TN; ++b) bf[b] = sB[buf][kk + l4][wn * 16 * TN + b * 16 + l15];
            double asum[TM], bsum[TN];
            if (M3) {
#pragma unroll
                for (int a = 0; a < TM; ++a) asum[a] = af[a].x + af[a].y;
#pragma unroll
                for (int b = 0; b < TN; ++b) bsum[b] = bf[b].x + bf[b].y;
            }
#pragma unroll
            for (int a = 0; a < TM; ++a)
#pragma unroll
                for (int b = 0; b < TN; ++b) {
                    if (M3) {
                        acc_re[a][b] = __builtin_amdgcn_mfma_f64_16x16x4f64(bf[b].x, af[a].x, acc_re[a][b], 0, 0, 0);
                        acc_p2[a][b] = __builtin_amdgcn_mfma_f64_16x16x4f64(bf[b].y, af[a].y, acc_p2[a][b], 0, 0, 0);
                        acc_im[a][b] = __builtin_amdgcn_mfma_f64_16x16x4f64(bsum[b], asum[a], acc_im[a][b], 0, 0, 0);
                    } else {
                        acc_re[a][b] = __builtin_amdgcn_mfma_f64_16x16x4f64(bf[b].x, af[a].x, acc_re[a][b], 0, 0, 0);
                        acc_re[a][b] = __builtin_amdgcn_mfma_f64_16x16x4f64(-bf[b].y, af[a].y, acc_re[a][b], 0, 0, 0);
                        acc_im[a][b] = __builtin_amdgcn_mfma_f64_16x16x4f64(bf[b].y, af[a].x, acc_im[a][b], 0, 0, 0);
                        acc_im[a][b] = __builtin_amdgcn_mfma_f64_16x16x4f64(bf[b].x, af[a].y, acc_im[a][b], 0, 0, 0);
                    }
                }
        }
    };
    const int Mm1 = g.M - 1, Nm1 = g.N - 1;

    if constexpr (FULL != 0) {
    constexpr bool GATHER = FULL == 2;
    constexpr double csgnA = OPA ? -1.0 : 1.0, csgnB = OPB ? -1.0 : 1.0;
    const int kbeg = g.b_lower ? (j0 / BK) * BK : 0;
    const int last = (K - kbeg) / BK - 1;
    const cplx *baseA, *baseB;
    unsigned offA, offB;
    size_t esA, ssA, esB, ssB;
    if (!OPA) { baseA = g.A + (size_t)kbeg * g.lda + i0; offA = (unsigned)(tid / BM) * g.lda + tid % BM; esA = (size_t)(256 / BM) * g.lda; ssA = (size_t)BK * g.lda; }
    else      { baseA = g.A + (size_t)i0 * g.lda + kbeg; offA = (unsigned)(tid / BK) * g.lda + tid % BK; esA = (size_t)(256 / BK) * g.lda; ssA = BK; }
    if (!OPB) { baseB = g.B + (size_t)j0 * g.ldb + kbeg; offB = (unsigned)(tid / BK) * g.ldb + tid % BK; esB = (size_t)(256 / BK) * g.ldb; ssB = BK; }
    else      { baseB = g.B + (size_t)kbeg * g.ldb + j0; offB = (unsigned)(tid / BN) * g.ldb + tid % BN; esB = (size_t)(256 / BN) * g.ldb; ssB = (size_t)BK * g.ldb; }
    int cnext[GATHER ? NA : 1];
    auto gidx = [&](int s) {
        if constexpr (GATHER) {
            const int* kg = g.a_kgather + kbeg + min(s, last) * BK + tid / BM;
// ... 118 lines not shown
                rb[e] = g.B[(size_t)min(gk, Km1) * g.ldb + min(gj, Nm1)];
                okb[e] = gj < g.N && gk < K;
            }
        }
    };
    auto sstore = [&](int buf) {
        constexpr double csgnA = OPA ? -1.0 : 1.0, csgnB = OPB ? -1.0 : 1.0;
#pragma unroll
        for (int e = 0; e < NA; ++e) {
            const int idx = tid + e * 256;
            int i, k;
            if (!OPA) { i = idx % BM; k = idx / BM; } else { k = idx % BK; i = idx / BK; }
            cplx v = make_double2(ra[e].x, csgnA * ra[e].y);
            if (has_kscale) { const double f = g.kscale_invert ? 1.0 / rsc[e] : rsc[e]; v.x *= f; v.y *= f; }
            if (!oka[e]) v = make_double2(0.0, 0.0);
            sA[buf][k][i] = v;
        }
#pragma unroll
        for (int e = 0; e < NB_; ++e) {
            const int idx = tid + e * 256;
            int j, k;
            if (!OPB) { k = idx % BK; j = idx / BK; } else { j = idx % BN; k = idx / BN; }
            sB[buf][k][j] = okb[e] ? make_double2(rb[e].x, csgnB * rb[e].y) : make_double2(0.0, 0.0);
        }
    };

    const int kbeg = g.ksplit > 1 ? kslice0 : (g.b_lower ? (j0 / BK) * BK : 0);
    if (K > kbeg) { gidx(kbeg); gload(kbeg); sstore(0); }
    __syncthreads();
    for (int k0 = kbeg, buf = 0; k0 < K; k0 += BK, buf ^= 1) {
        const bool more = k0 + BK < K;
        if (more) gload(k0 + BK);
        __builtin_amdgcn_sched_barrier(0);
        mfma_tile(buf);
        __builtin_amdgcn_sched_barrier(0);
        if (more) sstore(buf ^ 1);
        __syncthreads();
    }
    }

#pragma unroll
    for (int a = 0; a < TM; ++a)
#pragma unroll
        for (int b = 0; b < TN; ++b) {
            const int gi = i0 + wm * 16 * TM + a * 16 + l15;
            const int gic = FULL ? gi : min(gi, Mm1);
            cplx cold[4];
            if (g.accumulate && g.csrc.X) {
                int col[4];
#pragma unroll
                for (int r = 0; r < 4; ++r) {
                    const int gj = j0 + wn * 16 * TN + b * 16 + l4 + 4 * r;
                    const int gjc = FULL ? gj : min(gj, Nm1);
                    col[r] = g.csrc.idx ? g.csrc.idx[gjc] : gjc;
                }
#pragma unroll
                for (int r = 0; r < 4; ++r) cold[r] = g.csrc.X[(size_t)col[r] * g.csrc.ld + gic];
#pragma unroll
                for (int r = 0; r < 4; ++r) cold[r] = col_src_value(cold[r], g.csrc.scale ? g.csrc.scale[col[r]] : 1.0);
            } else if (g.accumulate) {
#pragma unroll
                for (int r = 0; r < 4; ++r) {
                    const int gj = j0 + wn * 16 * TN + b * 16 + l4 + 4 * r;
                    cold[r] = g.C[(size_t)(FULL ? gj : min(gj, Nm1)) * g.ldc + gic];
                }
            }
#pragma unroll
            for (int r = 0; r < 4; ++r) {
                const int gj = j0 + wn * 16 * TN + b * 16 + l4 + 4 * r;
                double re = acc_re[a][b][r], im = acc_im[a][b][r];
                if (M3) { const double p1 = re, p2 = acc_p2[a][b][r]; re = p1 - p2; im = (im - p1) - p2; }
                if (!FULL && g.ksplit > 1) {
                    if (gi < g.M && gj < g.N) g.part[((size_t)blockIdx.y * g.N + gj) * g.M + gi] = make_double2(re, im);
                    continue;
                }
                const int gjc = FULL ? gj : min(gj, Nm1);
                if (g.rowscale) { double sc = g.rowscale[gic]; if (g.colscale) sc *= g.colscale[gjc]; re *= sc; im *= sc; }
                else if (g.colscale) { double sc = g.colscale[gjc]; re *= sc; im *= sc; }
                if (g.negate) { re = -re; im = -im; }
                if (g.accumulate) { re += cold[r].x; im += cold[r].y; }
                if (FULL || (gi < g.M && gj < g.N)) g.C[(size_t)gj * g.ldc + gi] = make_double2(re, im);
            }
        }
}

template<bool M3, bool FULL, int STAGE, int TAG>
__global__ __launch_bounds__(256, (FULL && STAGE == 1) ? 3 : 2) void k_flush(const cplx* __restrict__ X, const cplx* __restrict__ GrT, int ld,
                                                  cplx* __restrict__ G, int ldc, int n, int Kmax, const int* __restrict__ Kdev,
                                                  int Kmul, size_t cs, int nb, const int* __restrict__ skip) {
    const int tn = (n + 63) / 64;
    int chain, tile;
    xcd_chain_tile(tn * tn, nb, chain, tile);
    X = chain_ptr_i(X, cs, chain); GrT = chain_ptr_i(GrT, cs, chain); G = chain_ptr_i(G, cs, chain); Kdev = chain_ptr_i(Kdev, cs, chain);
    skip = chain_ptr_i(skip, cs, chain);
    if (skip && *skip) return;
    int K = Kmax;
    if (Kdev) { int kd = (*Kdev) * Kmul; K = kd < K ? kd : K; }
    if (K <= 0) return;
    const int K8 = (K + 7) & ~7;
    const int tid = threadIdx.x, lane = tid & 63, wave = tid >> 6;
    const int l15 = lane & 15, l4 = lane >> 4;
    const int i0 = (tile % tn) * 64 + (wave >> 1) * 32, j0 = (tile / tn) * 64 + (wave & 1) * 32;
    if (i0 >= n || j0 >= n) return;
    v4d acc_re[2][2], acc_im[2][2], acc_p2[M3 ? 2 : 1][M3 ? 2 : 1];
#pragma unroll
    for (int a = 0; a < 2; ++a)
#pragma unroll
        for (int b = 0; b < 2; ++b) { acc_re[a][b] = (v4d)(0.0); acc_im[a][b] = (v4d)(0.0); if (M3) acc_p2[a][b] = (v4d)(0.0); }
    const int ia = FULL ? i0 + l15 : min(i0 + l15, n - 1), ia2 = FULL ? ia + 16 : min(i0 + 16 + l15, n - 1);
    const int jb = FULL ? j0 + l15 : min(j0 + l15, n - 1), jb2 = FULL ? jb + 16 : min(j0 + 16 + l15, n - 1);
    const cplx* xa = X + (size_t)l4 * ld;
    const cplx* gb = GrT + (size_t)l4 * ld;
    auto loadf = [&](int k0, cplx (&f)[4]) {
        const size_t o = (size_t)k0 * ld;
        f[0] = xa[o + ia]; f[1] = xa[o + ia2]; f[2] = gb[o + jb]; f[3] = gb[o + jb2];
    };
    auto mac = [&](const cplx (&f)[4]) {
        double asum[2], bsum[2];
        if (M3) {
#pragma unroll
            for (int a = 0; a < 2; ++a) { asum[a] = f[a].x + f[a].y; bsum[a] = f[2 + a].x + f[2 + a].y; }
        }
#pragma unroll
        for (int a = 0; a < 2; ++a)
#pragma unroll
            for (int b = 0; b < 2; ++b) {
                if (M3) {
                    acc_re[a][b] = __builtin_amdgcn_mfma_f64_16x16x4f64(f[2 + b].x, f[a].x, acc_re[a][b], 0, 0, 0);
                    acc_p2[a][b] = __builtin_amdgcn_mfma_f64_16x16x4f64(f[2 + b].y, f[a].y, acc_p2[a][b], 0, 0, 0);
                    acc_im[a][b] = __builtin_amdgcn_mfma_f64_16x16x4f64(bsum[b], asum[a], acc_im[a][b], 0, 0, 0);
                } else {
                    acc_re[a][b] = __builtin_amdgcn_mfma_f64_16x16x4f64(f[2 + b].x, f[a].x, acc_re[a][b], 0, 0, 0);
                    acc_re[a][b] = __builtin_amdgcn_mfma_f64_16x16x4f64(-f[2 + b].y, f[a].y, acc_re[a][b], 0, 0, 0);
                    acc_im[a][b] = __builtin_amdgcn_mfma_f64_16x16x4f64(f[2 + b].y, f[a].x, acc_im[a][b], 0, 0, 0);
                    acc_im[a][b] = __builtin_amdgcn_mfma_f64_16x16x4f64(f[2 + b].x, f[a].y, acc_im[a][b], 0, 0, 0);
                }
            }
    };
    if constexpr (STAGE == 1) {
        cplx s[4], t[4];
        loadf(0, s);
        for (int k0 = 0; k0 < K8; k0 += 8) {
            loadf(k0 + 4, t);
            __builtin_amdgcn_sched_barrier(0);
            mac(s);
            __builtin_amdgcn_sched_barrier(0);
            loadf(min(k0 + 8, K8 - 4), s);
            __builtin_amdgcn_sched_barrier(0);
            mac(t);
            __builtin_amdgcn_sched_barrier(0);
        }
    } else {
        cplx s0[4], s1[4], t0[4], t1[4];
        loadf(0, s0);
        loadf(4, s1);
        for (int k0 = 0; k0 < K8; k0 += 16) {
            const int kn = min(k0 + 8, K8 - 8);
            loadf(kn, t0);
            loadf(kn + 4, t1);
            __builtin_amdgcn_sched_barrier(0);
            mac(s0);
            mac(s1);
            __builtin_amdgcn_sched_barrier(0);
            if (k0 + 8 >= K8) break;
            const int kn2 = min(k0 + 16, K8 - 8);
            loadf(kn2, s0);
// ... 230 lines not shown
}

template<int TM, int TN, bool M3, int TAG, int FULL>
static void launch_gemm_ops(const Launch& lc, const GemmArgs& a, dim3 grid) {
    if (!a.opA) {
        if (!a.opB) hipLaunchKernelGGL((k_zgemm<TM, TN, M3, TAG, false, false, FULL>), grid, dim3(256), 0, lc.st, a, lc.cs, lc.nb);
        else        hipLaunchKernelGGL((k_zgemm<TM, TN, M3, TAG, false, true, FULL>), grid, dim3(256), 0, lc.st, a, lc.cs, lc.nb);
    } else if constexpr (FULL != 2) {
        if (!a.opB) hipLaunchKernelGGL((k_zgemm<TM, TN, M3, TAG, true, false, FULL>), grid, dim3(256), 0, lc.st, a, lc.cs, lc.nb);
        else        hipLaunchKernelGGL((k_zgemm<TM, TN, M3, TAG, true, true, FULL>), grid, dim3(256), 0, lc.st, a, lc.cs, lc.nb);
    }
}
GemmPlan gemm_plan(const GemmArgs& a, int nb) {
    GemmPlan p;
    p.xcd = nb % 8 == 0;
    p.ksplit = 1;
    const long tiles64 = (long)((a.M + 63) / 64) * ((a.N + 63) / 64) * nb;
    if (tiles64 >= 256 && a.N > 32 && a.M > 32) { p.tile = 64; return p; }
    p.tile = 32;
    const long wg = (long)((a.M + 31) / 32) * ((a.N + 31) / 32) * nb;
    if (a.part && a.K >= 512 && !a.Kdev && !a.kscale && !a.rowscale && !a.colscale && !a.b_lower && wg < 256) {
        const long cap = (long)((a.part_count ? a.part_count : (size_t)a.M * a.N * 8) / ((size_t)a.M * a.N));
        const int ks = (int)std::min<long>(std::min<long>(std::min<long>(32, cap), a.K / 64), (512 + wg - 1) / wg);
        if (ks >= 2) p.ksplit = ks;
    }
    return p;
}

static int gemm_full_path(const GemmArgs& a, const GemmPlan& p) {
    if (p.ksplit > 1 || use_4m() || a.M <= 0 || a.N <= 0 || a.M % p.tile || a.N % p.tile || a.K < 16 || a.K % 16 || a.Kdev || a.kscale) return 0;
    if (a.b_lower && a.K < a.N) return 0;
    if (a.lda < 1 || a.ldb < 1 || a.lda > (1 << 22) || a.ldb > (1 << 22)) return 0;
    const bool gather = a.a_kgather && !a.opA;
    if (gather && a.tag) return 0;
    return gather ? 2 : 1;
}

template<int TAG>
static int launch_gemm_tagged(const Launch& lc, const GemmArgs& a, int path) {
    const GemmPlan p = gemm_plan(a, lc.nb);
    const int t = ((a.M + p.tile - 1) / p.tile) * ((a.N + p.tile - 1) / p.tile);
    dim3 grid = p.xcd ? dim3(t * lc.nb, 1, 1) : dim3(t, 1, lc.nb);
    int full = path == 0 ? 0 : gemm_full_path(a, p);
    if (full == 2 && TAG != 0) full = 0;
    if (full == 1) {
        if (p.tile == 64) launch_gemm_ops<2, 2, true, TAG, 1>(lc, a, grid);
        else              launch_gemm_ops<1, 1, true, TAG, 1>(lc, a, grid);
        return 1;
    }
    if constexpr (TAG == 0) {
        if (full == 2) {
            if (p.tile == 64) launch_gemm_ops<2, 2, true, 0, 2>(lc, a, grid);
            else              launch_gemm_ops<1, 1, true, 0, 2>(lc, a, grid);
            return 1;
        }
    }
    if (p.tile == 64) {
        if (use_4m() && TAG == 0) launch_gemm_ops<2, 2, false, 0, 0>(lc, a, grid);
        else                      launch_gemm_ops<2, 2, true, TAG, 0>(lc, a, grid);
    } else if (p.ksplit > 1) {
        GemmArgs g2 = a;
        g2.ksplit = p.ksplit; g2.accumulate = 0; g2.negate = 0;
        grid.y = p.ksplit;
        launch_gemm_ops<1, 1, true, TAG, 0>(lc, g2, grid);
        hipLaunchKernelGGL(k_gemm_reduce, dim3(std::min(256, (a.M * a.N + 255) / 256), 1, lc.nb), dim3(256), 0, lc.st, a.part, p.ksplit, a.M, a.N,
                           a.C, a.ldc, a.accumulate, a.negate, lc.cs);
    } else {
        if (use_4m() && TAG == 0) launch_gemm_ops<1, 1, false, 0, 0>(lc, a, grid);
        else                      launch_gemm_ops<1, 1, true, TAG, 0>(lc, a, grid);
    }
    return 0;
}
int launch_gemm_path(const Launch& lc, const GemmArgs& a, int path) {
    int ran;
    if (a.tag) {
        if (lc.sub) lc.sub->begin(lc.sub->user, SUBFAM_FACT_GEMM);
        ran = launch_gemm_tagged<1>(lc, a, path);
        if (lc.sub) lc.sub->end(lc.sub->user, SUBFAM_FACT_GEMM, 8.0 * a.M * a.N * a.K * lc.nb,
                                16.0 * ((double)a.M * a.K + (double)a.K * a.N + (a.accumulate ? 2.0 : 1.0) * a.M * a.N) * lc.nb);
    } else ran = launch_gemm_tagged<0>(lc, a, path);
    return ran;
}
void launch_gemm(const Launch& lc, const GemmArgs& a) { (void)launch_gemm_path(lc, a, -1); }
```

detqmc_amd/csrc/kernels_qr.hip:

```cpp
#include "dqmc_internal.h"
#include <cstring>

#define QR_NB 16

template<int CTRL, int ROWMASK>
__device__ __forceinline__ double q_dpp_add(double v) {
    int lo = __double2loint(v), hi = __double2hiint(v);
    int lo2 = __builtin_amdgcn_update_dpp(0, lo, CTRL, ROWMASK, 0xf, false);
    int hi2 = __builtin_amdgcn_update_dpp(0, hi, CTRL, ROWMASK, 0xf, false);
    return v + __hiloint2double(hi2, lo2);
}
__device__ __forceinline__ double q_readlane_d(double x, int l) {
    int lo = __builtin_amdgcn_readlane(__double2loint(x), l);
    int hi = __builtin_amdgcn_readlane(__double2hiint(x), l);
    return __hiloint2double(hi, lo);
}
__device__ __forceinline__ double q_wave_total(double v) {
    v = q_dpp_add<0xB1, 0xf>(v);
    v = q_dpp_add<0x4E, 0xf>(v);
    v = q_dpp_add<0x114, 0xf>(v);
    v = q_dpp_add<0x118, 0xf>(v);
    v = q_dpp_add<0x142, 0xa>(v);
    v = q_dpp_add<0x143, 0xc>(v);
    return q_readlane_d(v, 63);
// ... 559 lines not shown
            panel(p + 1);
            apply(true, A, p, j0 + 2 * QR_NB, 2 * QR_NB, p, 1, 2);
            panel(p + 2);
            apply(true, A, p + 2, j0 + 3 * QR_NB, QR_NB, p + 2, 1, 1);
            panel(p + 3);
            apply(true, A, p, j0 + 4 * QR_NB, left - 4 * QR_NB, p, 1, 4);
            p += 4;
        } else if (reg && left > 2 * QR_NB) {
            panel(p);
            apply(true, A, p, j0 + QR_NB, QR_NB, p, 1, 1);
            panel(p + 1);
            apply(true, A, p, j0 + 2 * QR_NB, left - 2 * QR_NB, p, 1, 2);
            p += 2;
        } else {
            panel(p);
            const int ntrail = left - nbof(p);
            if (ntrail > 0) apply(true, A, p, j0 + nbof(p), ntrail, p, 1, 1);
            p += 1;
        }
    }
    if (!Q) return launches;
    launch_set_identity(lc, Q, n);
    ++launches;
    for (int p = np - 1; p >= 0;) {
        int cnt = 1;
        if (reg && nbof(p) == QR_NB) cnt = (p >= 3) ? 4 : (p >= 1 ? 2 : 1);
        const int lo = p - (cnt - 1);
        apply(false, Q, lo, lo * QR_NB, n - lo * QR_NB, p, -1, cnt);
        p -= cnt;
    }
    return launches;
}

int run_qr_apply_q(const Launch& lc, int n, cplx* C, const QrWork& w, int trans) {
    int launches = 0;
    const int np = (n + QR_NB - 1) / QR_NB;
    const bool reg = n <= 512;
    auto nbof = [&](int p) { return (n - p * QR_NB < QR_NB) ? (n - p * QR_NB) : QR_NB; };
    auto group = [&](int first, int step, int cnt, int lo) {
        const int rows = n - lo * QR_NB;
        cplx* Cs = C + lo * QR_NB;
        const dim3 grid((n + QR_NB - 1) / QR_NB, 1, lc.nb);
        if (w.apply_hooks) w.apply_hooks->begin(w.apply_hooks->user);
        if (reg) {
            QrRefs r;
            r.n = cnt;
            for (int i = 0; i < QR_MAXREF; ++i) { r.V[i] = nullptr; r.Tn[i] = nullptr; r.nb[i] = 0; }
            for (int i = 0; i < cnt; ++i) {
                const int q = first + i * step;
                r.V[i] = w.V + (size_t)(q * QR_NB) * n + lo * QR_NB;
                r.Tn[i] = w.T + (size_t)q * 2 * QR_NB * QR_NB + QR_NB * QR_NB;
                r.nb[i] = nbof(q);
            }
            if (trans) launch_apply_reg<true>(lc, grid, r, n, Cs, n, rows, n);
            else       launch_apply_reg<false>(lc, grid, r, n, Cs, n, rows, n);
        } else {
            const cplx* Vq = w.V + (size_t)(first * QR_NB) * n + lo * QR_NB;
            const cplx* Tq = w.T + (size_t)first * 2 * QR_NB * QR_NB + QR_NB * QR_NB;
            if (trans) hipLaunchKernelGGL((k_qr_apply<true>), grid, dim3(256), 0, lc.st, Vq, n, Tq, Cs, n, rows, n, nbof(first), lc.cs);
            else       hipLaunchKernelGGL((k_qr_apply<false>), grid, dim3(256), 0, lc.st, Vq, n, Tq, Cs, n, rows, n, nbof(first), lc.cs);
        }
        if (w.apply_hooks) w.apply_hooks->end(w.apply_hooks->user, 1);
        ++launches;
    };
    if (trans) {
        for (int p = 0; p < np;) {
            int cnt = 1;
            if (reg) { cnt = (np - p >= 4) ? 4 : ((np - p >= 2) ? 2 : 1); if (nbof(p + cnt - 1) != QR_NB) cnt = 1; }
            group(p, 1, cnt, p);
            p += cnt;
        }
    } else {
        for (int p = np - 1; p >= 0;) {
            int cnt = 1;
            if (reg && nbof(p) == QR_NB) cnt = (p >= 3) ? 4 : (p >= 1 ? 2 : 1);
            group(p, -1, cnt, p - (cnt - 1));
            p -= cnt;
        }
    }
    return launches;
}

#define TRSM_NB 32
__global__ __launch_bounds__(256) void k_trsm_block(cplx* __restrict__ C, int ldc, const cplx* __restrict__ R, int ldr,
                                                     int n, int j0, int nb, int trans, int unit, size_t cs, ColSrc S) {
    __shared__ cplx sR[TRSM_NB][TRSM_NB + 1];
    CHAIN(C); CHAIN(R); CHAIN(S.X); CHAIN(S.idx); CHAIN(S.scale);
    for (int i = threadIdx.x; i < TRSM_NB * TRSM_NB; i += 256) {
        int r = i % TRSM_NB, c = i / TRSM_NB;
        cplx v = make_double2(0.0, 0.0);
        if (r < nb && c < nb && r <= c) {
            if (unit && r == c) v = make_double2(1.0, 0.0);
            else if (trans) { const cplx t = R[(size_t)(j0 + r) * ldr + (j0 + c)]; v = make_double2(t.x, -t.y); }
            else v = R[(size_t)(j0 + c) * ldr + (j0 + r)];
        }
        if (r == c && r < nb) {
            v = cplx_recip(v);
        }
        sR[r][c] = v;
    }
    __syncthreads();
    int row = blockIdx.x * 256 + threadIdx.x;
    if (row >= n) return;
    cplx y[TRSM_NB];
    if (S.X) {
        int col[TRSM_NB];
#pragma unroll
        for (int c = 0; c < TRSM_NB; ++c) { const int jc = j0 + min(c, nb - 1); col[c] = S.idx ? S.idx[jc] : jc; }
#pragma unroll
        for (int c = 0; c < TRSM_NB; ++c) y[c] = S.X[(size_t)col[c] * S.ld + row];
#pragma unroll
        for (int c = 0; c < TRSM_NB; ++c) y[c] = col_src_value(y[c], S.scale ? S.scale[col[c]] : 1.0);
    } else {
#pragma unroll
        for (int c = 0; c < TRSM_NB; ++c) y[c] = C[(size_t)(j0 + min(c, nb - 1)) * ldc + row];
    }
#pragma unroll
    for (int c = 0; c < TRSM_NB; ++c) {
        if (c < nb) {
            cplx acc = y[c];
#pragma unroll
            for (int k = 0; k < TRSM_NB; ++k) {
                if (k < c) {
                    cplx t = q_cmul(y[k], sR[k][c]);
                    acc.x -= t.x; acc.y -= t.y;
                }
            }
            y[c] = q_cmul(acc, sR[c][c]);
        }
    }
#pragma unroll
    for (int c = 0; c < TRSM_NB; ++c)
        if (c < nb) C[(size_t)(j0 + c) * ldc + row] = y[c];
}

__global__ void k_negate_copy_block(const cplx* __restrict__ R, int ldr, int rows, int cols, cplx* __restrict__ out, int ldo, size_t cs) {
    CHAIN(R); CHAIN(out);
    size_t total = (size_t)rows * cols;
    for (size_t idx = blockIdx.x * (size_t)blockDim.x + threadIdx.x; idx < total; idx += (size_t)gridDim.x * blockDim.x) {
        int i = (int)(idx % rows), j = (int)(idx / rows);
        cplx v = R[(size_t)j * ldr + i];
        out[(size_t)j * ldo + i] = make_double2(-v.x, -v.y);
    }
}

static int trsm_rec(const Launch& lc, int n, const cplx* R, cplx* C, int j0, int len, int trans, int unit, const ColSrc* src = nullptr) {
    const ColSrc none = ColSrc();
    if (len <= TRSM_NB) {
        hipLaunchKernelGGL(k_trsm_block, dim3((n + 255) / 256, 1, lc.nb), dim3(256), 0, lc.st, C, n, R, n, n, j0, len, trans, unit, lc.cs,
                           src ? col_src_from(*src, j0) : none);
        return 1;
    }
    const int h = ((len / 2 + TRSM_NB - 1) / TRSM_NB) * TRSM_NB;
    int launches = trsm_rec(lc, n, R, C, j0, h, trans, unit, src);
    GemmArgs g = GemmArgs();
    g.A = C + (size_t)j0 * n; g.lda = n; g.opA = 0; g.C = C + (size_t)(j0 + h) * n; g.ldc = n;
    if (trans) { g.B = R + (size_t)j0 * n + (j0 + h); g.ldb = n; g.opB = 1; }
    else       { g.B = R + (size_t)(j0 + h) * n + j0; g.ldb = n; g.opB = 0; }
    g.M = n; g.N = len - h; g.K = h; g.Kmul = 1; g.accumulate = 1; g.negate = 1; g.tag = 1;
    if (src) g.csrc = col_src_from(*src, j0 + h);
    launch_gemm(lc, g);
    launches += 1;
    return launches + trsm_rec(lc, n, R, C, j0 + h, len - h, trans, unit);
}
int run_trsm_right_upper(const Launch& lc, int n, const cplx* R, cplx* C, const QrWork& w, int trans, int unit, const ColSrc* src) {
    (void)w;
    if (src && (!src->X || src->X == C)) src = nullptr;
    return trsm_rec(lc, n, R, C, 0, n, trans, unit, src);
}

#define BGS_NB 64
#define CHOL_PIVOT_TOL 1e-12
#define CHOL_NQ 16
__global__ __launch_bounds__(64 * CHOL_NQ) void k_chol64(cplx* __restrict__ Gm, int ld, int j0, int nb, cplx* __restrict__ R1m, int* __restrict__ err, size_t cs) {
    __shared__ cplx s[BGS_NB][BGS_NB + 1];
    __shared__ cplx s1[BGS_NB][BGS_NB + 1];
    __shared__ cplx prow[2][BGS_NB];
    CHAIN(Gm); CHAIN(R1m); CHAIN(err);
    const int j = threadIdx.x & 63, q = __builtin_amdgcn_readfirstlane(threadIdx.x >> 6);
    constexpr int NS = BGS_NB / CHOL_NQ;
    cplx a[NS], r1[NS];
#pragma unroll
    for (int t = 0; t < NS; ++t) {
        const int i = CHOL_NQ * t + q;
        const bool in = j < nb && i <= j;
        a[t] = in ? Gm[(size_t)(j0 + j) * ld + (j0 + i)] : make_double2(0.0, 0.0);
        r1[t] = (in && R1m) ? R1m[(size_t)(j0 + j) * ld + (j0 + i)] : make_double2(0.0, 0.0);
    }
    if (R1m) {
#pragma unroll
        for (int t = 0; t < NS; ++t) s1[CHOL_NQ * t + q][j] = r1[t];
    }
    if (q == 0) prow[0][j] = a[0];
    double g_orig = 1.0;
#pragma unroll
    for (int t = 0; t < NS; ++t) if (CHOL_NQ * t + q == j && j < nb) g_orig = a[t].x;
    for (int K = 0; K < nb; ++K) {
        __syncthreads();
        const cplx* pr = prow[K & 1];
        cplx pi[NS];
#pragma unroll
        for (int t = 0; t < NS; ++t) pi[t] = pr[CHOL_NQ * t + q];
        const cplx pj = pr[j];
        const double dkk = pr[K].x;
        if (j == K && (K & (CHOL_NQ - 1)) == q && err && !(dkk > CHOL_PIVOT_TOL * g_orig)) *err = 1;
        const double dk = fmax(dkk, 1e-300), id = rsqrt(dk), d = dk * id;
        const cplx rkj = make_double2(pj.x * id, pj.y * id);
        cplx pub = make_double2(0.0, 0.0);
#pragma unroll
        for (int t = 0; t < NS; ++t) {
            const int i = CHOL_NQ * t + q;
            if (i > K) {
                if (i <= j && j < nb) {
                    const cplx rki = make_double2(pi[t].x * id, pi[t].y * id);
                    a[t].x -= rki.x * rkj.x + rki.y * rkj.y;
                    a[t].y -= rki.x * rkj.y - rki.y * rkj.x;
                }
                if (i == K + 1) pub = a[t];
            } else if (i == K) {
                if (j >= K && j < nb) a[t] = (j == K) ? make_double2(d, 0.0) : rkj;
            }
        }
        if (((K + 1) & (CHOL_NQ - 1)) == q) prow[(K + 1) & 1][j] = pub;
    }
    __syncthreads();
#pragma unroll
    for (int t = 0; t < NS; ++t) {
        const int i = CHOL_NQ * t + q;
        s[i][j] = a[t];
        if (j < nb && i < nb) Gm[(size_t)(j0 + j) * ld + (j0 + i)] = (i <= j) ? a[t] : make_double2(0.0, 0.0);
    }
    if (!R1m) return;
    __syncthreads();
    cplx acc[NS];
#pragma unroll
    for (int u = 0; u < NS; ++u) acc[u] = make_double2(0.0, 0.0);
    for (int t = 0; t < nb; ++t) {
        const cplx b = s1[t][j];
#pragma unroll
        for (int u = 0; u < NS; ++u) {
            const int i = CHOL_NQ * u + q;
            if (i <= t) {
                const cplx x = s[i][t];
                if (t <= j) {
                    acc[u].x += x.x * b.x - x.y * b.y;
                    acc[u].y += x.x * b.y + x.y * b.x;
                }
            }
        }
    }
#pragma unroll
// ... 162 lines not shown
```

detqmc_amd/model.py:

```python
import ctypes as C
import re
from dataclasses import dataclass

import numpy as np

from . import _lib
from ._lib import check, load

BC = {"pbc": 0, "apbc-x": 1, "apbc-y": 2, "apbc-xy": 3}
UPDATE_METHOD = {"iterative": 0, "woodbury": 1, "delayed": 2}
STABILISATION = {"svd": 0, "qr": 1}
LEFT, RIGHT = 0, 1
UP, DOWN = +1, -1


@dataclass
class SDWParams:
    opdim: int = 2
    L: int = 4
    beta: float = 0.0
    m: int = 0
    dtau: float = 0.1
    s: int = 10
    r: float = -1.0
    c: float = 3.0
    u: float = 1.0
    lambda_: float = 1.0
    txhor: float = -1.0
    txver: float = -0.5
    tyhor: float = 0.5
    tyver: float = 1.0
    mu: float = -0.5
    mux: float = None
    muy: float = None
    accRatio: float = 0.5
    delaySteps: int = 16
    updateMethod: str = "delayed"
    bc: str = "pbc"
    weakZflux: bool = False
    globalShift: bool = False
    wolffClusterUpdate: bool = False
    wolffClusterShiftUpdate: bool = False
    repeatWolffPerSweep: int = 1
    fermionMeasurements: bool = False
    equalTimeCorrelators: bool = False
    timeDisplacedMeasurements: bool = False
    timeDisplacedPairing: bool = False
    timeDisplacedParticleHole: bool = False
    timeDisplacedCurrent: bool = False
    timeDisplacedEverySlice: bool = False
    bandCorrelators: bool = False
    timeDisplacedFineOnDevice: bool = False
    globalUpdateInterval: int = 100
    phi2bosons: bool = False
    cdwU: float = 0.0
    rngSeed: int = 1020304050
    simindex: int = 0
    device: int = 0
    stabilisation: str = "svd"
    checkerboard: bool = True
    spinProposalMethod: str = "box"
    adaptScaleVariance: bool = False
    repeatUpdateInSlice: int = 1
    pipeline: int = 0
    qrVariant: int = 0
    greenVariant: int = 0
    maxJacobiSweeps: int = 0
    proposalBudget: int = 0
    decideThreads: int = 0
    bmultPath: int = 0
    rngLookahead: int = 0


OBSERVABLES = {"kOccX": 0, "kOccY": 1, "pairPlus": 2, "pairMinus": 3, "greenKTauX": 4, "greenKTauY": 5,
               "pairPlusTau": 6, "pairMinusTau": 7, "pairPlusTauQ0": 8, "pairMinusTauQ0": 9,
               "chargeTau": 10, "spinZTau": 11, "sdwTau": 12, "chargeTauQ0": 13, "spinZTauQ0": 14, "sdwTauQ0": 15,
               "currentXTau": 16, "currentYTau": 17, "currentXTauQ0": 18, "currentYTauQ0": 19, "bondKineticX": 20, "bondKineticY": 21,
               "chargeCorr": 22, "spinZCorr": 23, "sdwCorr": 24, "pairPlusCorr": 25, "pairMinusCorr": 26,
               "chargeSq": 27, "spinZSq": 28, "sdwSq": 29, "pairPlusSq": 30, "pairMinusSq": 31, "phiChi": 32, "phiScalars": 33,
               "bandDiffTau": 34, "bandMixTau": 35, "bandDiffTauQ0": 36, "bandMixTauQ0": 37,
               "bandDiffCorr": 38, "bandMixCorr": 39, "bandDiffSq": 40, "bandMixSq": 41, "greenMatrixTau": 74}
MATSUBARA = {n: OBSERVABLES[n] for n in "greenKTauX greenKTauY pairPlusTau pairMinusTau chargeTau spinZTau sdwTau currentXTau currentYTau bandDiffTau bandMixTau".split()}
EQ_CORRELATORS = {n: OBSERVABLES[n] for n in "chargeCorr spinZCorr sdwCorr pairPlusCorr pairMinusCorr chargeSq spinZSq sdwSq pairPlusSq pairMinusSq".split()}
BAND_EQ_CORRELATORS = {n: OBSERVABLES[n] for n in "bandDiffCorr bandMixCorr bandDiffSq bandMixSq".split()}
SERIES_PHI_OBS = {n: OBSERVABLES[n] for n in "phiChi phiScalars".split()}
GREEN_MATRIX_OBS = OBSERVABLES["greenMatrixTau"]


def structure_factor(c, L):
    c = np.asarray(c, dtype=np.float64)
    L = int(L)
    x = np.arange(L * L) % L
    y = np.arange(L * L) // L
    ph = 2.0 * np.pi / L * (np.outer(x, x) + np.outer(y, y))
    return c @ np.cos(ph).T


def superfluid_stiffness(chi_xx, chi_yy, L):
    xx, yy = np.asarray(chi_xx)[..., 0, :], np.asarray(chi_yy)[..., 0, :]
    return 0.125 * np.real(xx[..., 1] - xx[..., L] + yy[..., L] - yy[..., 1])


SERIES_DERIVED = {"R_charge": 0, "R_spinZ": 1, "R_sdw": 2, "R_pairPlus": 3, "R_pairMinus": 4, "rhoS": 5,
                  "binderPhi": 6, "binderRatioPhi": 7, "chiPhi": 8, "chiPhiConnected": 9, "R_phi": 10, "xiPhi": 11,
                  "R_dCDW": 12, "R_nematic": 13, "R_bandMix": 14}
SERIES_EQ, SERIES_MATS_G, SERIES_MATS_PAIR, SERIES_MATS_PH, SERIES_MATS_CURRENT = 1, 2, 4, 8, 16
SERIES_PHI = 64
SERIES_MATS_BAND, SERIES_EQ_BAND = 128, 256
SERIES_MATS_CUSTOM, SERIES_EQ_CUSTOM = 512, 1024
CUSTOM_OBS_BASE = {"Tau": 42, "TauQ0": 46, "Corr": 50, "Sq": 54}


def custom_observable(name):
    m = re.fullmatch(r"custom([0-3])(Tau|TauQ0|Corr|Sq)", name)
    return (m.group(2), CUSTOM_OBS_BASE[m.group(2)] + int(m.group(1))) if m else None


def custom_ratio(name):
    m = re.fullmatch(r"R_custom([0-3])", name)
    return int(m.group(1)) if m else None


SERIES_MATS_CUSTOM_PAIR, SERIES_EQ_CUSTOM_PAIR = 2048, 4096
CUSTOM_PAIR_OBS_BASE = {"Tau": 58, "TauQ0": 62, "Corr": 66, "Sq": 70}


def custom_pair_observable(name):
    m = re.fullmatch(r"customPair([0-3])(Tau|TauQ0|Corr|Sq)", name)
    return (m.group(2), CUSTOM_PAIR_OBS_BASE[m.group(2)] + int(m.group(1))) if m else None


def custom_pair_ratio(name):
    m = re.fullmatch(r"R_customPair([0-3])", name)
    return int(m.group(1)) if m else None


SERIES_GREEN_MATRIX = 8192
PAIR_VERTEX_QUANTITIES = {"vertexCustomPair": 0, "bubbleCustomPair": 1, "gammaCustomPair": 2, "gammaBubbleCustomPair": 3}


def pair_vertex_quantity(name):
    m = re.fullmatch(r"(vertexCustomPair|bubbleCustomPair|gammaCustomPair|gammaBubbleCustomPair)([0-3])", name)
    return (PAIR_VERTEX_QUANTITIES[m.group(1)], int(m.group(2))) if m else None


PH_VERTEX_QUANTITIES = {"vertexCustom": 0, "bubbleCustom": 1, "gammaCustom": 2, "gammaBubbleCustom": 3, "disconnectedCustom": 4}


def ph_vertex_quantity(name):
    m = re.fullmatch(r"(vertexCustom|bubbleCustom|gammaCustom|gammaBubbleCustom|disconnectedCustom)([0-3])", name)
    return (PH_VERTEX_QUANTITIES[m.group(1)], int(m.group(2))) if m else None


def observable_index(name):
# ... 51 lines not shown
    mean = x.sum(axis=0) / B
    loo = (B * mean - x) / (B - 1)
    if f is None:
        return mean, np.sqrt((B - 1) / B * ((loo - mean) ** 2).sum(axis=0))
    theta = np.array([f(v) for v in loo])
    return f(mean), np.sqrt((B - 1) / B * ((theta - theta.sum(axis=0) / B) ** 2).sum(axis=0))


def binning_analysis(bins, bin_size, variance=None):
    y = np.asarray(bins, dtype=np.float64)
    if y.shape[0] < 2:
        raise ValueError("the binning analysis needs at least two bins")
    errs, taus = [], []
    if variance is not None:
        var = np.asarray(variance, dtype=np.float64)
        safe = np.where(var > 0, var, 1.0)
    level = 0
    while y.shape[0] >= 2:
        errs.append(jackknife(y)[1])
        if variance is not None:
            t = 0.5 * errs[-1] * errs[-1] * (float(y.shape[0]) * float(1 << level) * float(bin_size)) / safe
            taus.append(np.where(var > 0, t, np.nan))
        half = y.shape[0] // 2
        y = (y[0:2 * half:2] + y[1:2 * half:2]) * 0.5
        level += 1
    return np.array(errs) if variance is None else (np.array(errs), np.array(taus))


GREEN_CHECK_FIELDS = ("count", "lastMaxAbs", "maxAbs", "sumMaxAbs", "maxSiteDiag", "sumMeanAbs", "maxRel", "argmax", "nonfinite",
                      "logScaleSpread", "logSvSpread")


def green_check_decode(raw, ng):
    raw = np.asarray(raw, dtype=np.float64)
    if raw.ndim != 4 or raw.shape[1] != 2 or raw.shape[3] != len(GREEN_CHECK_FIELDS):
        raise ValueError("green_check_decode: expected shape (chains, 2, n+1, %d), got %r" % (len(GREEN_CHECK_FIELDS), raw.shape))
    f = {name: raw[..., i] for i, name in enumerate(GREEN_CHECK_FIELDS)}
    count = f["count"].astype(np.int64)
    denom = np.maximum(count, 1)
    idx = f["argmax"].astype(np.int64)
    return {"count": count, "lastMaxAbs": f["lastMaxAbs"].copy(), "maxAbs": f["maxAbs"].copy(), "meanMaxAbs": f["sumMaxAbs"] / denom,
            "maxSiteDiag": f["maxSiteDiag"].copy(), "meanAbs": f["sumMeanAbs"] / denom, "maxRel": f["maxRel"].copy(),
            "argmax": np.stack([idx % ng, idx // ng], axis=-1), "nonfinite": f["nonfinite"].astype(np.int64),
            "logScaleSpread": f["logScaleSpread"].copy(), "logSvSpread": f["logSvSpread"].copy()}


def green_check_worst(decoded):
    out = []
    for mx, am in zip(decoded["maxAbs"], decoded["argmax"]):
        d, j = np.unravel_index(int(np.argmax(mx)), mx.shape)
        out.append((float(mx[d, j]), int(d), int(j), int(am[d, j, 0]), int(am[d, j, 1])))
    return out


class _GreenCheck:

    def _gc_handle(self):
        return self.h

    def set_green_check(self, on=True):
        check(getattr(self.lib, self._gc_calls[0])(self._gc_handle(), int(on)), host=self._gc_calls[3])

    def _green_check_raw(self):
        chains, n, _ = self._gc_shape()
        raw = np.zeros((chains, 2, n + 1, len(GREEN_CHECK_FIELDS)))
        check(getattr(self.lib, self._gc_calls[1])(self._gc_handle(), raw.ctypes.data_as(_lib._DP)), host=self._gc_calls[3])
        return raw

    def green_check(self):
        return green_check_decode(self._green_check_raw(), self._gc_shape()[2])

    def green_check_worst(self):
        return green_check_worst(self.green_check())

    def green_check_reset(self):
        check(getattr(self.lib, self._gc_calls[2])(self._gc_handle()), host=self._gc_calls[3])


SPIN_PROPOSAL = {"box": 0, "rotate_then_scale": 1, "rotate_and_scale": 2}
PROPOSE = {"box": 0, "rotate": 1, "scale": 2, "rotate_and_scale": 3}
ADAPT = {"box": 0, "rotate": 1, "scale": 2}


def _tuning(pipeline=0, qrVariant=0, greenVariant=0, maxJacobiSweeps=0, proposalBudget=0, decideThreads=0, bmultPath=0, rngLookahead=0):
    if int(rngLookahead) not in (0, -1):
        raise ValueError("rngLookahead must be 0 (automatic: on) or -1 (off)")
    path = int(bmultPath) | (_lib.DQMC_TUNING_NO_RNG_LOOKAHEAD if int(rngLookahead) == -1 and 0 <= int(bmultPath) <= 2 else 0)
    return _lib.dqmc_tuning(pipeline=int(pipeline), qr_variant=int(qrVariant), green_variant=int(greenVariant),
                            max_jacobi_sweeps=int(maxJacobiSweeps), proposal_budget=int(proposalBudget),
                            decide_threads=int(decideThreads), bmult_path=path)


def _fmat(a):
    return np.array(a, dtype=np.complex128, order="F", copy=True)


def _custom_matrices(mats):
    return np.ascontiguousarray(np.asarray(list(mats), dtype=np.complex128).reshape(-1, 4, 4))


def _custom_bond_operators(ops):
    ops = [tuple(op) for op in ops]
    if any(len(op) != 3 for op in ops):
        raise ValueError("every operator is a tuple (M0, Mx, My); None stands for a zero matrix")
    zero = np.zeros((4, 4), dtype=np.complex128)
    return [_custom_matrices([zero if op[k] is None else op[k] for op in ops]) for k in range(3)]


def _get_custom_bond(call, handle, host):
    n = C.c_int(0)
    m = [np.zeros((_lib.DQMC_CUSTOM_MAX, 4, 4), dtype=np.complex128) for _ in range(3)]
    check(call(handle, C.byref(n), *[a.ctypes.data for a in m]), host=host)
    return [tuple(a[c].copy() for a in m) for c in range(n.value)]


def _bond_tuple(params, mu, factor):
    mu = {"x": 0, "y": 1}.get(mu, mu)
    if mu not in (0, 1):
        raise ValueError("mu must be 'x' or 'y' (0 or 1)")
    hop = ((params.txhor, params.tyhor), (params.txver, params.tyver))[mu]
    M = factor * np.diag([-hop[0], -hop[1], -hop[0], -hop[1]]).astype(np.complex128)
    return (None, M, None) if mu == 0 else (None, None, M)


def bond_current(params, mu):
    return _bond_tuple(params, mu, 1j)


def bond_kinetic(params, mu):
    return _bond_tuple(params, mu, 1.0)


def pair_operator(kind):
    XUP, YDOWN, XDOWN, YUP = 0, 1, 2, 3
    F = np.zeros((4, 4), dtype=np.complex128)
    if kind in ("s", "d_band"):
        F[XUP, XDOWN], F[YUP, YDOWN] = 1.0, 1.0 if kind == "s" else -1.0
        return (F, None, None)
    if kind in ("s_ext", "d_bond"):
        F[XUP, XDOWN] = F[YUP, YDOWN] = 1.0
        F[XDOWN, XUP] = F[YDOWN, YUP] = -1.0
        return (None, F, F.copy() if kind == "s_ext" else -F)
    raise ValueError("kind must be 's', 'd_band', 's_ext' or 'd_bond'")


def pair_bubble(gbar, ops, L, bc="pbc"):
    g = np.asarray(gbar, dtype=np.complex128)
    N, R = L * L, g.shape[-1]
    if bc not in ("pbc", "apbc-x", "apbc-y", "apbc-xy") or g.shape[-3:] != (N, R, R) or R not in (2, 4):
        raise ValueError("gbar must be (..., L L, R, R) with R = 2 or 4, bc one of 'pbc', 'apbc-x', 'apbc-y', 'apbc-xy'")
    apb = (bc in ("apbc-x", "apbc-xy"), bc in ("apbc-y", "apbc-xy"))
    if R == 2:
        full = np.zeros(g.shape[:-2] + (4, 4), dtype=np.complex128)
        full[..., :2, :2] = g
        full[..., 2:, 2:] = np.conj(g)
        g = full
    ax, ay = np.arange(N) % L, np.arange(N) // L
    zero = np.zeros((4, 4), dtype=np.complex128)

    def block(px, py, qx, qy):
        dx, dy = (px - qx) % L, (py - qy) % L
        sg = np.where(apb[0] & (qx + dx >= L), -1.0, 1.0) * np.where(apb[1] & (qy + dy >= L), -1.0, 1.0)
        return sg[:, None, None] * g[..., dy * L + dx, :, :]

    PA = [(ax, ay, np.ones(N)), ((ax + 1) % L, ay, np.where(apb[0] & (ax == L - 1), -1.0, 1.0)), (ax, (ay + 1) % L, np.where(apb[1] & (ay == L - 1), -1.0, 1.0))]
    QB = [(0, 0), (1 % L, 0), (0, 1 % L)]
    out = []
    for op in ops:
        F = [zero if m is None else np.asarray(m, dtype=np.complex128) for m in op]
        acc = np.zeros(g.shape[:-3] + (N,))
        for ka in range(3):
            if not F[ka].any():
                continue
            px, py, ua = PA[ka]
            for kb in range(3):
                if not F[kb].any():
                    continue
                qx, qy = QB[kb]
                direct = np.einsum("ab,cd,...ac,...bd->...", F[ka], np.conj(F[kb]), block(px, py, qx, qy), block(ax, ay, 0, 0), optimize=True)
                exchange = np.einsum("ab,cd,...ad,...bc->...", F[ka], np.conj(F[kb]), block(px, py, 0, 0), block(ax, ay, qx, qy), optimize=True)
                acc = acc + ua * (direct - exchange).real
        out.append(acc)
    return np.stack(out, axis=-2) if out else np.zeros(g.shape[:-3] + (0, N))


def _ph_full(gbar, L, bc, lead):
    g = np.asarray(gbar, dtype=np.complex128)
    N, R = L * L, g.shape[-1]
    if bc not in ("pbc", "apbc-x", "apbc-y", "apbc-xy") or g.ndim < 3 + lead or g.shape[-3:] != (N, R, R) or R not in (2, 4):
        raise ValueError("gbar must be (..., L L, R, R) with R = 2 or 4, bc one of 'pbc', 'apbc-x', 'apbc-y', 'apbc-xy'")
    if R == 2:
        full = np.zeros(g.shape[:-2] + (4, 4), dtype=np.complex128)
        full[..., :2, :2] = g
        full[..., 2:, 2:] = np.conj(g)
        g = full
    return g, (bc in ("apbc-x", "apbc-xy"), bc in ("apbc-y", "apbc-xy"))


def _ph_block(g, L, apb, P, Q):
    dx, dy = (P[0] - Q[0]) % L, (P[1] - Q[1]) % L
    sg = np.where(apb[0] & (Q[0] + dx >= L), -1.0, 1.0) * np.where(apb[1] & (Q[1] + dy >= L), -1.0, 1.0)
    return sg[:, None, None] * g[..., dy * L + dx, :, :]


def _ph_stencil(op, L, apb, sx, sy):
    zero = np.zeros((4, 4), dtype=np.complex128)
    M0, Mx, My = (zero if m is None else np.asarray(m, dtype=np.complex128) for m in op)
    S, Sx, Sy = (sx, sy), ((sx + 1) % L, sy), (sx, (sy + 1) % L)
    ux, uy = np.where(apb[0] & (sx == L - 1), -1.0, 1.0), np.where(apb[1] & (sy == L - 1), -1.0, 1.0)
    blocks = [(M0, S, S, np.ones(len(sx))), (Mx, Sx, S, ux), (Mx.conj().T, S, Sx, ux), (My, Sy, S, uy), (My.conj().T, S, Sy, uy)]
    return [b for b in blocks if b[0].any()]


def ph_bubble(gbar, ops, L, bc="pbc"):
    g, apb = _ph_full(gbar, L, bc, 1)
    N = L * L
    gt = -np.flip(g, axis=-4)
    ax, ay = np.arange(N) % L, np.arange(N) // L
    zx = np.zeros(N, dtype=int)
    out = []
    for op in ops:
        acc = np.zeros(g.shape[:-3] + (N,))
        for WA, pA, qA, fA in _ph_stencil(op, L, apb, ax, ay):
            for WB, rB, sB, fB in _ph_stencil(op, L, apb, zx, zx):
                tr = np.einsum("ab,...bc,cd,...da->...", WA, _ph_block(g, L, apb, qA, rB), WB, _ph_block(gt, L, apb, sB, pA), optimize=True)
                acc = acc - fA * fB * tr.real
        out.append(acc)
    return np.stack(out, axis=-2) if out else np.zeros(g.shape[:-3] + (0, N))


def ph_one_body(gbar0, ops, L, bc="pbc"):
    g, apb = _ph_full(gbar0, L, bc, 0)
    z = np.zeros(1, dtype=int)
    out = []
    for op in ops:
        M0 = np.zeros((4, 4), dtype=np.complex128) if op[0] is None else np.asarray(op[0], dtype=np.complex128)
        acc = np.trace(M0) + np.zeros(g.shape[:-3], dtype=np.complex128)
        for W, p, q, f in _ph_stencil(op, L, apb, z, z):
            acc = acc - f[0] * np.einsum("ab,...ba->...", W, _ph_block(g, L, apb, q, p)[..., 0, :, :])
        out.append(acc)
    return np.stack(out, axis=-1) if out else np.zeros(g.shape[:-3] + (0,), dtype=np.complex128)


class KernelContext:

    def __init__(self, opdim, L, m, s, dtau, delaySteps=16, bc="pbc", weakZflux=False, r=-1.0, c=3.0, u=1.0,
                 lambda_=1.0, txhor=-1.0, txver=-0.5, tyhor=0.5, tyver=1.0, mux=-0.5, muy=-0.5,
                 accRatio=0.5, phi2bosons=False, device=0, stabilisation="svd", checkerboard=True, nchains=1, cdwU=0.0,
                 pipeline=0, qrVariant=0, greenVariant=0, maxJacobiSweeps=0, proposalBudget=0, rngWindowPerSite=0, decideThreads=0, bmultPath=0,
                 rngLookahead=0, timeDisplaced=False, tdParticleHole=False, tdCurrent=False, tdEverySlice=False, tdBand=False):
        self.lib = load()
        p = _lib.dqmc_params(opdim=opdim, L=L, m=m, s=s, delaySteps=delaySteps, bc=BC[bc],
                             weakZflux=int(weakZflux), phi2bosons=int(phi2bosons), device=device,
                             stabilisation=STABILISATION[stabilisation], cb_none=int(not checkerboard), dtau=dtau, r=r, c=c, u=u, lambda_=lambda_, txhor=txhor, txver=txver,
                             tyhor=tyhor, tyver=tyver, mux=mux, muy=muy, accRatio=accRatio, cdwU=cdwU, rng_window_per_site=int(rngWindowPerSite),
                             timedisplaced=int(timeDisplaced) | (_lib.DQMC_TD_EVERY_SLICE if tdEverySlice else 0), td_particle_hole=(2 if tdCurrent else int(tdParticleHole)) | (_lib.DQMC_TD_PH_BAND if tdBand else 0),
                             tuning=_tuning(pipeline, qrVariant, greenVariant, maxJacobiSweeps, proposalBudget, decideThreads, bmultPath, rngLookahead))
        h = C.c_void_p()
        check(self.lib.dqmc_create_batch(C.byref(p), nchains, C.byref(h)))
        self.h = h
        self.nchains = nchains
        self.opdim, self.L, self.m, self.s = opdim, L, m, s
        self.N = L * L
        self.MSF = 4 if opdim == 3 else 2
        self.ng = self.MSF * self.N
        self.n = -(-m // s)

    def close(self):
        if self.h:
            self.lib.dqmc_destroy(self.h)
            self.h = None

    def __del__(self):
        try:
            self.close()
        except Exception:
            pass

    def shiftGreenSymmetric(self):
        g = np.zeros((self.ng, self.ng), dtype=np.complex128, order="F")
        check(self.lib.dqmc_shift_green_symmetric_host(self.h, g.ctypes.data))
        return g

    def set_timedisplaced(self, on=True):
        check(self.lib.dqmc_set_timedisplaced(self.h, int(on)))

    def green_timedisplaced(self):
        gt0 = np.zeros((self.ng, self.ng), dtype=np.complex128, order="F")
        g0t = np.zeros_like(gt0)
        sl = C.c_int(-1)
        check(self.lib.dqmc_get_green_timedisplaced_host(self.h, gt0.ctypes.data, g0t.ctypes.data, C.byref(sl)))
        return sl.value, gt0, g0t

    def _read_block(self, size_fn, read_fn, *which):
        out = np.zeros(size_fn(self.h, *which))
        check(read_fn(self.h, *which, out.ctypes.data_as(_lib._DP)))
        return out

    def measure_reset(self):
        check(self.lib.dqmc_measure_reset(self.h))

    def measure_slice(self):
        check(self.lib.dqmc_measure_slice(self.h))

    def measure_read(self):
        return self._read_block(self.lib.dqmc_measure_accum_size, self.lib.dqmc_measure_read_host)

    def set_equal_time_correlators(self, on=True):
        check(self.lib.dqmc_set_equal_time_correlators(self.h, int(on)))

    def measure_eq_read(self):
        return self._read_block(self.lib.dqmc_measure_eq_accum_size, self.lib.dqmc_measure_eq_read_host)

    def set_equal_time_band(self, on=True):
        check(self.lib.dqmc_set_equal_time_band(self.h, int(on)))

    def measure_eq_band_read(self):
        return self._read_block(self.lib.dqmc_measure_eq_band_accum_size, self.lib.dqmc_measure_eq_band_read_host)

    def hubbard_set_equal_time_correlators(self, on=True):
        check(self.lib.dqmc_hubbard_set_equal_time_correlators(self.h, int(on)))

    def hubbard_eq_read(self):
        return self._read_block(self.lib.dqmc_hubbard_eq_accum_size, self.lib.dqmc_hubbard_eq_read_host)

    def hubbard_measure_timedisplaced(self, j):
        check(self.lib.dqmc_hubbard_measure_timedisplaced(self.h, j))

    def hubbard_td_read(self):
        return self._read_block(self.lib.dqmc_hubbard_td_accum_size, self.lib.dqmc_hubbard_td_read_host)

    def measure_timedisplaced(self, j):
        check(self.lib.dqmc_measure_timedisplaced(self.h, j))

    def measure_td_read(self):
        return self._read_block(self.lib.dqmc_measure_td_accum_size, self.lib.dqmc_measure_td_read_host)

    def measure_timedisplaced_pair(self, j):
        check(self.lib.dqmc_measure_timedisplaced_pair(self.h, j))

# ... 468 lines not shown
        nb = self.nchains_total()
        a = np.zeros((nb, self.m + 1, self.opdim, self.N))
        check(self.lib.dqmc_get_fields_all_host(self.h, a.ctypes.data_as(_lib._DP)))
        return np.transpose(a, (0, 1, 3, 2)).copy()

    def sv_all(self):
        a = np.zeros((self.nchains_total(), self.ng))
        check(self.lib.dqmc_get_sv_all_host(self.h, a.ctypes.data_as(_lib._DP)))
        return a

    def nchains_total(self):
        return self.lib.dqmc_num_chains(self.h)

    def synchronize(self):
        check(self.lib.dqmc_synchronize(self.h))

    def schedule_info(self):
        si = _lib.dqmc_schedule_info()
        check(self.lib.dqmc_get_schedule_info(self.h, C.byref(si)))
        return si

    def profile_enable(self, on=True):
        check(self.lib.dqmc_profile_enable(self.h, int(on)))

    def profile_read(self):
        pr = _lib.dqmc_profile()
        check(self.lib.dqmc_profile_read(self.h, C.byref(pr)))
        names = ["bmult", "gemm", "decomp", "decide", "other", "gather", "flush"]
        out = {nm: (pr.ms[i], int(pr.launches[i])) for i, nm in enumerate(names)}
        out["jacobi"] = out["decomp"]
        out.update(svd_calls=int(pr.svd_calls), svd_sweeps_total=int(pr.svd_sweeps_total),
                   svd_sweeps_max=int(pr.svd_sweeps_max), qr_calls=int(pr.qr_calls), gemm_flops=pr.gemm_flops,
                   decomp_round_ms=pr.decomp_round_ms, decomp_rounds=int(pr.decomp_rounds),
                   blocks_nonempty=int(pr.blocks_nonempty), chains=int(pr.chains),
                   updates_accepted=int(pr.updates_accepted), lu_calls=int(pr.lu_calls),
                   sub={"lu_update": [pr.sub_ms[0], int(pr.sub_launches[0]), pr.sub_flops[0], pr.sub_bytes[0]],
                        "fact_gemm": [pr.sub_ms[1], int(pr.sub_launches[1]), pr.sub_flops[1], pr.sub_bytes[1]]})
        return out


class _CtxView(KernelContext):

    def __init__(self, lib, handle, info):
        self.lib, self.h = lib, C.c_void_p(handle)
        self.opdim, self.L, self.m, self.s = info.opdim, info.L, info.m, info.s
        self.N, self.MSF, self.ng, self.n = info.N, info.MSF, info.n_g, info.n

    def close(self):
        self.h = None


def _host_params(pars: SDWParams):
    if pars.timeDisplacedPairing and not pars.timeDisplacedMeasurements:
        raise ValueError("timeDisplacedPairing needs timeDisplacedMeasurements")
    if pars.timeDisplacedParticleHole and not pars.timeDisplacedMeasurements:
        raise ValueError("timeDisplacedParticleHole needs timeDisplacedMeasurements")
    if pars.equalTimeCorrelators and not pars.fermionMeasurements:
        raise ValueError("equalTimeCorrelators needs fermionMeasurements")
    if pars.timeDisplacedCurrent and not pars.timeDisplacedParticleHole:
        raise ValueError("timeDisplacedCurrent needs timeDisplacedParticleHole")
    if pars.bandCorrelators and not (pars.timeDisplacedParticleHole or pars.equalTimeCorrelators):
        raise ValueError("bandCorrelators needs timeDisplacedParticleHole or equalTimeCorrelators")
    band_td = bool(pars.bandCorrelators and pars.timeDisplacedParticleHole)
    band_eq = bool(pars.bandCorrelators and pars.equalTimeCorrelators)
    return _lib.detsdw_params(
        opdim=pars.opdim, L=pars.L, m=pars.m, s=pars.s, delaySteps=pars.delaySteps,
        globalShift=int(pars.globalShift), globalUpdateInterval=pars.globalUpdateInterval,
        weakZflux=int(pars.weakZflux), phi2bosons=int(pars.phi2bosons), device=pars.device,
        simindex=pars.simindex, rngSeed=pars.rngSeed,
        has_mux_muy=int(pars.mux is not None and pars.muy is not None),
        updateMethod=UPDATE_METHOD[pars.updateMethod], bc=pars.bc.encode(),
        beta=pars.beta, dtau=pars.dtau, r=pars.r, c=pars.c, u=pars.u, lambda_=pars.lambda_,
        txhor=pars.txhor, txver=pars.txver, tyhor=pars.tyhor, tyver=pars.tyver,
        mu=pars.mu, mux=pars.mux or 0.0, muy=pars.muy or 0.0, accRatio=pars.accRatio, cdwU=pars.cdwU,
        stabilisation=STABILISATION[pars.stabilisation], cb_none=int(not pars.checkerboard),
        wolffClusterUpdate=int(pars.wolffClusterUpdate), wolffClusterShiftUpdate=int(pars.wolffClusterShiftUpdate),
        repeatWolffPerSweep=int(pars.repeatWolffPerSweep), fermionMeasurements=int(bool(pars.fermionMeasurements)) | (_lib.DETSDW_FM_EQ_CORRELATORS if pars.equalTimeCorrelators else 0)
        | (_lib.DETSDW_FM_EQ_BAND if band_eq else 0),
        spinProposalMethod=SPIN_PROPOSAL[pars.spinProposalMethod], adaptScaleVariance=int(pars.adaptScaleVariance),
        repeatUpdateInSlice=int(pars.repeatUpdateInSlice), timeDisplacedMeasurements=(2 if pars.timeDisplacedPairing else int(bool(pars.timeDisplacedMeasurements)))
        | (_lib.DETSDW_TD_EVERY_SLICE if pars.timeDisplacedEverySlice else 0)
        | (_lib.DETSDW_TD_FINE_ON_DEVICE if pars.timeDisplacedFineOnDevice else 0),
        timeDisplacedParticleHole=(2 if pars.timeDisplacedCurrent else int(bool(pars.timeDisplacedParticleHole))) | (_lib.DETSDW_TD_PH_BAND if band_td else 0),
        tuning=_tuning(pars.pipeline, pars.qrVariant, pars.greenVariant, pars.maxJacobiSweeps, pars.proposalBudget, pars.decideThreads, pars.bmultPath, pars.rngLookahead))


class DetSDW(_GreenCheck):

    def __init__(self, pars: SDWParams = None, _batch=None, _chain=0):
        self.lib = load()
        self._chain = _chain
        self._batch = _batch
        if _batch is not None:
            self.h = _batch.h
            self.pars = _batch.pars_list[_chain]
            return
        p = _host_params(pars)
        h = C.c_void_p()
        check(self.lib.detsdw_create(C.byref(p), C.byref(h)), host=True)
        self.h = h
        self.pars = pars

    def _sel(self):
        if self._batch is not None:
            check(self.lib.detsdw_select_chain(self.h, self._chain), host=True)

    def close(self):
        if self._batch is not None:
            self.h = None
            return
        if self.h:
            self.lib.detsdw_destroy(self.h)
            self.h = None

    def __del__(self):
        try:
            self.close()
        except Exception:
            pass

    _gc_calls = ("detsdw_set_green_check", "detsdw_get_green_check", "detsdw_reset_green_check", True)

    def _gc_handle(self):
        if self._batch is not None:
            raise RuntimeError("the wrap-error diagnostics belong to the whole batch: call them on the DetSDWBatch")
        return self.h

    def _gc_shape(self):
        i = self.info
        return 1, i.n, i.n_g

    def sweep(self, takeMeasurements=False):
        if self._batch is not None:
            raise RuntimeError("a chain of a batch cannot sweep on its own: call DetSDWBatch.sweep()")
        check(self.lib.detsdw_sweep(self.h, int(takeMeasurements)), host=True)

    def sweepThermalization(self):
        if self._batch is not None:
            raise RuntimeError("a chain of a batch cannot sweep on its own: call DetSDWBatch.sweepThermalization()")
        check(self.lib.detsdw_sweep_thermalization(self.h), host=True)

    @property
    def info(self):
        self._sel()
        i = _lib.detsdw_info()
        check(self.lib.detsdw_get_info(self.h, C.byref(i)), host=True)
        return i

    @property
    def observables(self):
        self._sel()
        o = _lib.detsdw_observables()
        check(self.lib.detsdw_get_observables(self.h, C.byref(o)), host=True)
        return o

    def observable_vector(self, name):
        self._sel()
        which, d = observable_index(name)
        if d.family == _lib.DETSDW_OBS_FAMILY_PHI:
            raise KeyError(name)
        shape, cplx = observable_shape(d, self.info)
        out = np.zeros(shape, dtype=np.complex128 if cplx else np.float64)
        check(self.lib.detsdw_get_observable_vector(self.h, which, out.ctypes.data_as(_lib._DP)), host=True)
        return out

    def matsubara(self, name, nfreq):
        self._sel()
# ... 471 lines not shown
```

include/dqmc_hip.h:

```cpp
#ifndef DQMC_HIP_H_
#define DQMC_HIP_H_

#include <stddef.h>
#include <stdint.h>

#ifdef __cplusplus
extern "C" {
#endif

typedef struct dqmc_ctx dqmc_ctx;

typedef struct dqmc_cplx { double re, im; } dqmc_cplx;

enum {
    DQMC_OK = 0,
    DQMC_EINVAL = -1,
    DQMC_EHIP = -2,
    DQMC_ENOCONV = -3,
    DQMC_ERNG = -4,
    DQMC_ENODEV = -5
};

enum { DQMC_BC_PBC = 0, DQMC_BC_APBC_X = 1, DQMC_BC_APBC_Y = 2, DQMC_BC_APBC_XY = 3 };
enum { DQMC_LEFT = 0, DQMC_RIGHT = 1 };
enum { DQMC_UP = +1, DQMC_DOWN = -1 };
enum { DQMC_STAB_SVD = 0, DQMC_STAB_QR = 1 };
enum { DQMC_MODEL_SDW = 0, DQMC_MODEL_HUBBARD = 1 };
enum { DQMC_TD_EVERY_SLICE = 0x100 };
enum { DQMC_TD_PH_BAND = 0x100 };

typedef struct dqmc_tuning {
    int32_t pipeline;
    int32_t qr_variant;
    int32_t green_variant;
    int32_t max_jacobi_sweeps;
    int32_t proposal_budget;
    int32_t decide_threads;
    int32_t bmult_path;
} dqmc_tuning;
enum { DQMC_TUNING_NO_RNG_LOOKAHEAD = 0x100 };

typedef struct dqmc_params {
    int32_t opdim;
    int32_t L;
    int32_t m;
    int32_t s;
    int32_t delaySteps;
    int32_t bc;
    int32_t weakZflux;
    int32_t phi2bosons;
    int32_t device;
    int32_t stabilisation;
    int32_t cb_none;
    int32_t model;
    double dtau, r, c, u, lambda;
    double txhor, txver, tyhor, tyver;
    double mux, muy;
    double accRatio;
    double cdwU;
    int32_t rng_window_per_site;
    int32_t timedisplaced;
    dqmc_tuning tuning;
    int32_t td_particle_hole;
} dqmc_params;

typedef struct dqmc_update_state {
    double phiDelta;
    double targetAccRatio;
    double lastAccRatio;
    double ra_runningAverage;
    double ra_values[100];
    int32_t ra_samplesAdded;
    int32_t ra_head;
    uint64_t rng_consumed;
    uint64_t rng_avail;
    int32_t error;
    int32_t reserved;
    double angleDelta, scaleDelta;
    double curminAngleDelta, curmaxAngleDelta, curminScaleDelta, curmaxScaleDelta;
    double rot_runningAverage;
    double rot_values[100];
    double scl_runningAverage;
    double scl_values[100];
    int32_t rot_samplesAdded, rot_head, scl_samplesAdded, scl_head;
} dqmc_update_state;

int dqmc_create(const dqmc_params* p, dqmc_ctx** out);
int dqmc_create_batch(const dqmc_params* p, int nchains, dqmc_ctx** out);
int dqmc_select_chain(dqmc_ctx* ctx, int chain);
int dqmc_num_chains(dqmc_ctx* ctx);
void dqmc_destroy(dqmc_ctx* ctx);
const char* dqmc_last_error(void);
int dqmc_synchronize(dqmc_ctx* ctx);
void* dqmc_stream(dqmc_ctx* ctx);

int dqmc_set_fields_host(dqmc_ctx* ctx, const double* phi);
int dqmc_get_fields_host(dqmc_ctx* ctx, double* phi, double* coshTermPhi, double* sinhTermPhi);
int dqmc_set_cdwl_host(dqmc_ctx* ctx, const int32_t* cdwl);
int dqmc_get_cdwl_host(dqmc_ctx* ctx, int32_t* cdwl);
int dqmc_set_fields_all_host(dqmc_ctx* ctx, const double* phi_all);
int dqmc_get_fields_all_host(dqmc_ctx* ctx, double* phi_all);

int dqmc_bmult_host(dqmc_ctx* ctx, int side, int inverse, int k2, int k1, dqmc_cplx* A);
int dqmc_bmult_src_host(dqmc_ctx* ctx, int side, int inverse, int k2, int k1, const dqmc_cplx* src, dqmc_cplx* out, dqmc_cplx* src_after);

int dqmc_udv_decompose_host(dqmc_ctx* ctx, const dqmc_cplx* M, dqmc_cplx* U, double* d, dqmc_cplx* V_t,
                            int* sweeps_used);
int dqmc_decompose_host(dqmc_ctx* ctx, const dqmc_cplx* M, const double* colscale, const double* rowscale, int kind,
                        const dqmc_cplx* Aold, dqmc_cplx* U, double* d, dqmc_cplx* V_t, int* sweeps_used);
int dqmc_green_from_factors_host(dqmc_ctx* ctx, const dqmc_cplx* U_l, const double* d_l, const dqmc_cplx* V_l,
                                 const dqmc_cplx* U_r, const double* d_r, const dqmc_cplx* V_r,
                                 dqmc_cplx* G, double* sv, dqmc_cplx* GT0, dqmc_cplx* G0T, dqmc_cplx* G00);
int dqmc_gemm_host(dqmc_ctx* ctx, int opA, int opB, const dqmc_cplx* A, const dqmc_cplx* B, dqmc_cplx* C);

int dqmc_udv_setup(dqmc_ctx* ctx);
int dqmc_advance(dqmc_ctx* ctx, int dir, int l);
int dqmc_wrap(dqmc_ctx* ctx, int dir, int k);
int dqmc_wrap_skip(dqmc_ctx* ctx, int dir, int k);
int dqmc_reset_storage0(dqmc_ctx* ctx);
enum { DQMC_GREEN_CHECK_FIELDS = 11 };
int dqmc_set_green_check(dqmc_ctx* ctx, int on);
size_t dqmc_green_check_size(dqmc_ctx* ctx);
int dqmc_green_check_read_host(dqmc_ctx* ctx, double* out);
int dqmc_green_check_reset(dqmc_ctx* ctx);

int dqmc_push_uniforms_host(dqmc_ctx* ctx, const double* u, size_t n);
int dqmc_push_uniforms_all_host(dqmc_ctx* ctx, const double* u, size_t n);
int dqmc_uniforms_staging_host(dqmc_ctx* ctx, double** buf, size_t* capacity);
int dqmc_stage_uniforms_tail_host(dqmc_ctx* ctx, const double* u, size_t n);
int dqmc_advance_uniforms(dqmc_ctx* ctx, const uint64_t* offset );
int dqmc_get_uniform_window_host(dqmc_ctx* ctx, double* out, size_t n);
int dqmc_update_slice(dqmc_ctx* ctx, int k, int thermalization);
enum { DQMC_PROPOSE_BOX = 0, DQMC_PROPOSE_ROTATE = 1, DQMC_PROPOSE_SCALE = 2, DQMC_PROPOSE_ROTATE_AND_SCALE = 3 };
enum { DQMC_ADAPT_BOX = 0, DQMC_ADAPT_ROTATE = 1, DQMC_ADAPT_SCALE = 2 };
int dqmc_update_slice_ex(dqmc_ctx* ctx, int k, int thermalization, int proposal, int adapt, int adapt_scale_variance, int repeat);
int dqmc_update_slice_final(dqmc_ctx* ctx, int k, int thermalization, int proposal, int adapt, int adapt_scale_variance, int repeat,
                            int then_wrap_dir);
typedef struct dqmc_schedule_info {
    int32_t pipelined;
    int32_t proposal_budget;
    uint64_t blocks_pipelined;
    uint64_t blocks_sequential;
    int32_t qr_block_gram_schmidt;
    int32_t green_lu;
    uint64_t cholqr_fallbacks;
    uint64_t uniform_windows_advanced;
    uint64_t uniform_windows_pushed;
} dqmc_schedule_info;
int dqmc_get_schedule_info(dqmc_ctx* ctx, dqmc_schedule_info* out);
int dqmc_get_update_state_host(dqmc_ctx* ctx, dqmc_update_state* out);
int dqmc_get_update_states_all_host(dqmc_ctx* ctx, dqmc_update_state* out );
int dqmc_set_update_state_host(dqmc_ctx* ctx, const dqmc_update_state* in);

int dqmc_get_green_host(dqmc_ctx* ctx, dqmc_cplx* out);
int dqmc_set_green_host(dqmc_ctx* ctx, const dqmc_cplx* in, int currentTimeslice);
int dqmc_get_sv_host(dqmc_ctx* ctx, double* out);
int dqmc_get_sv_all_host(dqmc_ctx* ctx, double* out );
int dqmc_get_udv_host(dqmc_ctx* ctx, int l, dqmc_cplx* U, double* d, dqmc_cplx* V_t);
int dqmc_current_timeslice(dqmc_ctx* ctx);

int dqmc_backup(dqmc_ctx* ctx);
int dqmc_restore(dqmc_ctx* ctx);
int dqmc_phi_action_all_host(dqmc_ctx* ctx, double* out);
int dqmc_shift_fields_all_host(dqmc_ctx* ctx, const double* shifts);
int dqmc_exchange_action_host(dqmc_ctx* ctx, double* out);
int dqmc_exchange_actions_device(dqmc_ctx* ctx, double* out_dev);

int dqmc_shift_green_symmetric_host(dqmc_ctx* ctx, dqmc_cplx* out);
int dqmc_measure_reset(dqmc_ctx* ctx);
int dqmc_measure_slice(dqmc_ctx* ctx);
size_t dqmc_measure_accum_size(dqmc_ctx* ctx);
int dqmc_measure_read_host(dqmc_ctx* ctx, double* out);
int dqmc_set_equal_time_correlators(dqmc_ctx* ctx, int on);
size_t dqmc_measure_eq_accum_size(dqmc_ctx* ctx);
int dqmc_measure_eq_read_host(dqmc_ctx* ctx, double* out);
int dqmc_set_equal_time_band(dqmc_ctx* ctx, int on);
size_t dqmc_measure_eq_band_accum_size(dqmc_ctx* ctx);
int dqmc_measure_eq_band_read_host(dqmc_ctx* ctx, double* out);
int dqmc_hubbard_set_equal_time_correlators(dqmc_ctx* ctx, int on);
size_t dqmc_hubbard_eq_accum_size(dqmc_ctx* ctx);
int dqmc_hubbard_eq_read_host(dqmc_ctx* ctx, double* out);
int dqmc_hubbard_measure_timedisplaced(dqmc_ctx* ctx, int j);
size_t dqmc_hubbard_td_accum_size(dqmc_ctx* ctx);
int dqmc_hubbard_td_read_host(dqmc_ctx* ctx, double* out);
int dqmc_set_timedisplaced(dqmc_ctx* ctx, int on);
int dqmc_get_green_timedisplaced_host(dqmc_ctx* ctx, dqmc_cplx* g_t0, dqmc_cplx* g_0t, int* slice);
int dqmc_measure_timedisplaced(dqmc_ctx* ctx, int j);
size_t dqmc_measure_td_accum_size(dqmc_ctx* ctx);
int dqmc_measure_td_read_host(dqmc_ctx* ctx, double* out);
int dqmc_measure_timedisplaced_pair(dqmc_ctx* ctx, int j);
size_t dqmc_measure_td_pair_accum_size(dqmc_ctx* ctx);
int dqmc_measure_td_pair_read_host(dqmc_ctx* ctx, double* out);
int dqmc_measure_timedisplaced_ph(dqmc_ctx* ctx, int j);
size_t dqmc_measure_td_ph_accum_size(dqmc_ctx* ctx);
int dqmc_measure_td_ph_read_host(dqmc_ctx* ctx, double* out);
int dqmc_measure_timedisplaced_current(dqmc_ctx* ctx, int j);
size_t dqmc_measure_td_current_accum_size(dqmc_ctx* ctx);
int dqmc_measure_td_current_read_host(dqmc_ctx* ctx, double* out);
int dqmc_measure_timedisplaced_band(dqmc_ctx* ctx, int j);
size_t dqmc_measure_td_band_accum_size(dqmc_ctx* ctx);
int dqmc_measure_td_band_read_host(dqmc_ctx* ctx, double* out);
#define DQMC_CUSTOM_MAX 4
int dqmc_set_custom_bilinears(dqmc_ctx* ctx, int count, const dqmc_cplx* M);
int dqmc_get_custom_bilinears(dqmc_ctx* ctx, int* count, dqmc_cplx* M);
int dqmc_measure_timedisplaced_custom(dqmc_ctx* ctx, int j);
size_t dqmc_measure_td_custom_accum_size(dqmc_ctx* ctx);
int dqmc_measure_td_custom_read_host(dqmc_ctx* ctx, double* out);
int dqmc_set_equal_time_custom(dqmc_ctx* ctx, int on);
size_t dqmc_measure_eq_custom_accum_size(dqmc_ctx* ctx);
int dqmc_measure_eq_custom_read_host(dqmc_ctx* ctx, double* out);
int dqmc_set_custom_bond_bilinears(dqmc_ctx* ctx, int count, const dqmc_cplx* M0, const dqmc_cplx* Mx, const dqmc_cplx* My);
int dqmc_get_custom_bond_bilinears(dqmc_ctx* ctx, int* count, dqmc_cplx* M0, dqmc_cplx* Mx, dqmc_cplx* My);
int dqmc_set_custom_pair_operators(dqmc_ctx* ctx, int count, const dqmc_cplx* F0, const dqmc_cplx* Fx, const dqmc_cplx* Fy);
int dqmc_get_custom_pair_operators(dqmc_ctx* ctx, int* count, dqmc_cplx* F0, dqmc_cplx* Fx, dqmc_cplx* Fy);
int dqmc_measure_timedisplaced_custom_pair(dqmc_ctx* ctx, int j);
size_t dqmc_measure_td_custom_pair_accum_size(dqmc_ctx* ctx);
int dqmc_measure_td_custom_pair_read_host(dqmc_ctx* ctx, double* out);
int dqmc_set_equal_time_custom_pair(dqmc_ctx* ctx, int on);
size_t dqmc_measure_eq_custom_pair_accum_size(dqmc_ctx* ctx);
int dqmc_measure_eq_custom_pair_read_host(dqmc_ctx* ctx, double* out);
int dqmc_set_green_matrix(dqmc_ctx* ctx, int on);
int dqmc_measure_timedisplaced_green_matrix(dqmc_ctx* ctx, int j);
size_t dqmc_measure_td_green_matrix_accum_size(dqmc_ctx* ctx);
int dqmc_measure_td_green_matrix_read_host(dqmc_ctx* ctx, double* out);
int dqmc_get_green0_timedisplaced_host(dqmc_ctx* ctx, dqmc_cplx* g00, int* slice);
int dqmc_measure_timedisplaced_segment(dqmc_ctx* ctx, int j);
int dqmc_measure_timedisplaced_ends(dqmc_ctx* ctx);
size_t dqmc_measure_td_fine_accum_size(dqmc_ctx* ctx, int channel);
int dqmc_measure_td_fine_read_host(dqmc_ctx* ctx, int channel, double* out);
size_t dqmc_measure_td_matsubara_size(dqmc_ctx* ctx, int channel, int nfreq);
// ... 63 lines not shown
```

Measured before the change: 299.6 sweeps/s.

## Batch left and right triangular solves into paired TRSM and GEMM launches

On the LU Green's-function route, the left and right half triangular solves share the same triangular factor. They are now issued together: each recursive TRSM block kernel and each trailing GEMM update handles both problems via blockIdx.y. This halves the number of kernel launches in the recursive solve and doubles the grid per launch, which should help the small n_g=512 problems fill the GPU. It adds a GEMM pair kernel with a runtime opB branch, and falls back to separate launches when the tiling plans of the two problems differ.

```diff
diff --git a/detqmc_amd/_lib.py b/detqmc_amd/_lib.py
--- a/detqmc_amd/_lib.py
+++ b/detqmc_amd/_lib.py
@@ -43,12 +43,14 @@
 
 
 DQMC_TUNING_NO_RNG_LOOKAHEAD = 0x100
+DQMC_TUNING_SINGLE_TRSM = 0x200
 
 
 class dqmc_schedule_info(C.Structure):
     _fields_ = [("pipelined", C.c_int32), ("proposal_budget", C.c_int32), ("blocks_pipelined", C.c_uint64),
                 ("blocks_sequential", C.c_uint64), ("qr_block_gram_schmidt", C.c_int32), ("green_lu", C.c_int32),
-                ("cholqr_fallbacks", C.c_uint64), ("uniform_windows_advanced", C.c_uint64), ("uniform_windows_pushed", C.c_uint64)]
+                ("cholqr_fallbacks", C.c_uint64), ("uniform_windows_advanced", C.c_uint64), ("uniform_windows_pushed", C.c_uint64),
+                ("trsm_paired", C.c_int32), ("reserved0", C.c_int32), ("trsm_pairs", C.c_uint64)]
 
 
 class dqmc_params(C.Structure):
diff --git a/detqmc_amd/csrc/dqmc_context.hip b/detqmc_amd/csrc/dqmc_context.hip
--- a/detqmc_amd/csrc/dqmc_context.hip
+++ b/detqmc_amd/csrc/dqmc_context.hip
@@ -335,7 +335,7 @@
     if (p->tuning.decide_threads != 0 && p->tuning.decide_threads != 256 && p->tuning.decide_threads != 512)
         return fail(DQMC_EINVAL, "tuning.decide_threads must be 0, 256 or 512");
     {
-        const int path = p->tuning.bmult_path & ~DQMC_TUNING_NO_RNG_LOOKAHEAD;
+        const int path = p->tuning.bmult_path & ~DQMC_TUNING_FLAG_BITS;
         if (p->tuning.bmult_path < 0 || path > 2) return fail(DQMC_EINVAL, "tuning.bmult_path must be 0, 1 or 2");
     }
     if (p->stabilisation != DQMC_STAB_SVD && p->stabilisation != DQMC_STAB_QR) return fail(DQMC_EINVAL, "stabilisation");
@@ -384,7 +384,7 @@
     if (p->tuning.proposal_budget != 0) hm.pbudget = p->tuning.proposal_budget < 0 ? 0 : p->tuning.proposal_budget;
     if (hm.pbudget > 0 && hm.pbudget < p->delaySteps) hm.pbudget = p->delaySteps;
     hm.decide_nt = p->tuning.decide_threads;
-    hm.bmult_path = p->tuning.bmult_path & ~DQMC_TUNING_NO_RNG_LOOKAHEAD;
+    hm.bmult_path = p->tuning.bmult_path & ~DQMC_TUNING_FLAG_BITS;
 #ifdef DQMC_DECIDE_TIMING
     hm.dbg = (getenv("DQMC_DECIDE_TIMING") && atoi(getenv("DQMC_DECIDE_TIMING"))) ? 8 : 0;
 #endif
@@ -480,6 +480,7 @@
     if (p->tuning.max_jacobi_sweeps > 0) c->max_jacobi_sweeps = p->tuning.max_jacobi_sweeps;
     c->qr_bgs = p->tuning.qr_variant == 2 || (p->tuning.qr_variant == 0 && ng > 1024);
     c->green_lu = ng <= 512 && p->tuning.green_variant != 1;
+    c->trsm_pair = c->green_lu && !(p->tuning.bmult_path & DQMC_TUNING_SINGLE_TRSM);
     if (c->stab == DQMC_STAB_QR) A_(alloc_qr_work(c));
     A_(alloc_slot(c, c->eye));
     const int WD = MSF * c->D;
@@ -883,6 +884,13 @@
     if (z.route == Z_QR_EXPLICIT) run_gemm(c, gemm_square(c, z.Q, 1, stage, 0, dst));
     return launches;
 }
+static int both_halves(dqmc_ctx* c, const ZFactors& z, const cplx* X, const double* xscale, cplx* A, const cplx* Yh, const double* yscale, cplx* B) {
+    ProfScope ps(c, FAM_JACOBI, 0);
+    const TrsmProblem left = {A, 0, 0, ColSrc{X, c->n_g, nullptr, xscale}};
+    const TrsmProblem right = {B, 1, 1, ColSrc{Yh, c->n_g, c->qr_perm, yscale}};
+    c->trsm_pairs += 1;
+    return run_trsm_right_upper_pair(c->lc, c->n_g, z.tri, left, right);
+}
 
 static int green_qr(dqmc_ctx* c, const UdVSlot* Lp, const UdVSlot* Rp, cplx* Gout, double* svout, bool td = false) {
     const UdVSlot& L = Lp ? *Lp : c->eye;
@@ -901,13 +909,20 @@
     ZFactors z;
     int launches = 0;
     { int rc = factorise_z(c, svout, &z, &launches); if (rc) return rc; }
-    launches += left_half(c, z, L.Vt, c->lmax_inv, c->T3);
-    launches += right_half(c, z, R.U, c->rmax_inv, c->T1, c->sw.V);
+    const bool paired = z.route == Z_LU && c->trsm_pair;
+    if (paired) launches += both_halves(c, z, L.Vt, c->lmax_inv, c->T3, R.U, c->rmax_inv, c->T1);
+    else {
+        launches += left_half(c, z, L.Vt, c->lmax_inv, c->T3);
+        launches += right_half(c, z, R.U, c->rmax_inv, c->T1, c->sw.V);
+    }
     if (Gout) run_gemm(c, gemm_square(c, c->T3, 0, c->T1, z.adjoint, Gout));
     if (td) {
         cplx* Bmin = z.route == Z_LU ? c->T4 : c->T2;
-        launches += right_half(c, z, R.Vt, c->rmin, Bmin, c->td_W);
-        launches += left_half(c, z, L.U, c->lmin, c->td_W);
+        if (paired) launches += both_halves(c, z, L.U, c->lmin, c->td_W, R.Vt, c->rmin, Bmin);
+        else {
+            launches += right_half(c, z, R.Vt, c->rmin, Bmin, c->td_W);
+            launches += left_half(c, z, L.U, c->lmin, c->td_W);
+        }
         run_gemm(c, gemm_square(c, c->T3, 0, Bmin, z.adjoint, c->GT0));
         g = gemm_square(c, c->td_W, 0, c->T1, z.adjoint, c->G0T);
         g.negate = 1;
@@ -1369,6 +1384,8 @@
     out->cholqr_fallbacks = c->cholqr_fallbacks;
     out->uniform_windows_advanced = c->windows_advanced;
     out->uniform_windows_pushed = c->windows_pushed;
+    out->trsm_paired = (c->stab == DQMC_STAB_QR && c->trsm_pair) ? 1 : 0;
+    out->trsm_pairs = c->trsm_pairs;
     return DQMC_OK;
 }
 
diff --git a/detqmc_amd/csrc/dqmc_ctx.h b/detqmc_amd/csrc/dqmc_ctx.h
--- a/detqmc_amd/csrc/dqmc_ctx.h
+++ b/detqmc_amd/csrc/dqmc_ctx.h
@@ -44,6 +44,8 @@
     bool pipelined = false;
     uint64_t blocks_pipelined = 0, blocks_sequential = 0, cholqr_fallbacks = 0;
     bool qr_bgs = false, green_lu = false;
+    bool trsm_pair = false;
+    uint64_t trsm_pairs = 0;
     std::vector<int> err_host;
     Launch lc{nullptr, 1, 0};
     int nb = 1, sel = 0;
diff --git a/detqmc_amd/csrc/dqmc_internal.h b/detqmc_amd/csrc/dqmc_internal.h
--- a/detqmc_amd/csrc/dqmc_internal.h
+++ b/detqmc_amd/csrc/dqmc_internal.h
@@ -154,6 +154,7 @@
 };
 void launch_gemm(const Launch& lc, const GemmArgs& a);
 int launch_gemm_path(const Launch& lc, const GemmArgs& a, int path);
+int launch_gemm_pair(const Launch& lc, const GemmArgs& a0, const GemmArgs& a1);
 struct GemmPlan { int tile, ksplit, xcd; };
 GemmPlan gemm_plan(const GemmArgs& a, int nb);
 void launch_flush(const Launch& lc, const cplx* X, const cplx* GrT, int ld, cplx* G, int ldc, int n, int Kmax,
@@ -310,6 +311,8 @@
 void qr_reset_workspace(const Launch& lc, int n, const QrWork& w);
 int run_trsm_right_upper(const Launch& lc, int n, const cplx* R, cplx* C, const QrWork& w, int trans = 0, int unit = 0,
                          const ColSrc* src = nullptr);
+struct TrsmProblem { cplx* C; int trans, unit; ColSrc src; };
+int run_trsm_right_upper_pair(const Launch& lc, int n, const cplx* R, const TrsmProblem& p0, const TrsmProblem& p1);
 #define LU_SWAP_INTS 128
 int run_lu(const Launch& lc, int n, cplx* A, int* perm, int* swaps, cplx* tneg);
 void launch_gather_scale_cols(const Launch& lc, const cplx* X, const double* cs, const int* perm, int n, cplx* Y);
diff --git a/detqmc_amd/csrc/kernels_gemm.hip b/detqmc_amd/csrc/kernels_gemm.hip
--- a/detqmc_amd/csrc/kernels_gemm.hip
+++ b/detqmc_amd/csrc/kernels_gemm.hip
@@ -5,12 +5,10 @@
 
 typedef double v4d __attribute__((ext_vector_type(4)));
 
-template<int TM, int TN, bool M3, int TAG, bool OPA, bool OPB, int FULL>
-__global__ __launch_bounds__(256, 2) void k_zgemm(GemmArgs g, size_t cs, int nb) {
+template<int TM, int TN, bool M3, bool OPA, bool OPB, int FULL>
+__device__ __forceinline__ void zgemm_body(GemmArgs g, size_t cs, int nb, cplx (&sA)[2][16][32 * TM + 1], cplx (&sB)[2][16][32 * TN + 1]) {
     constexpr int BM = 32 * TM, BN = 32 * TN, BK = 16;
     constexpr int NA = BM * BK / 256, NB_ = BN * BK / 256;
-    __shared__ cplx sA[2][BK][BM + 1];
-    __shared__ cplx sB[2][BK][BN + 1];
     const int tm = (g.M + BM - 1) / BM, tnn = (g.N + BN - 1) / BN;
     int chain, tile;
     xcd_chain_tile(tm * tnn, nb, chain, tile);
@@ -295,6 +293,23 @@
                 if (FULL || (gi < g.M && gj < g.N)) g.C[(size_t)gj * g.ldc + gi] = make_double2(re, im);
             }
         }
+}
+
+template<int TM, int TN, bool M3, int TAG, bool OPA, bool OPB, int FULL>
+__global__ __launch_bounds__(256, 2) void k_zgemm(GemmArgs g, size_t cs, int nb) {
+    __shared__ cplx sA[2][16][32 * TM + 1];
+    __shared__ cplx sB[2][16][32 * TN + 1];
+    zgemm_body<TM, TN, M3, OPA, OPB, FULL>(g, cs, nb, sA, sB);
+}
+
+struct GemmPair { GemmArgs g[2]; };
+template<int TM, int TN, bool M3, int TAG, int FULL>
+__global__ __launch_bounds__(256, 2) void k_zgemm_pair(GemmPair p, size_t cs, int nb) {
+    __shared__ cplx sA[2][16][32 * TM + 1];
+    __shared__ cplx sB[2][16][32 * TN + 1];
+    const GemmArgs& g = p.g[blockIdx.y ? 1 : 0];
+    if (g.opB) zgemm_body<TM, TN, M3, false, true, FULL>(g, cs, nb, sA, sB);
+    else       zgemm_body<TM, TN, M3, false, false, FULL>(g, cs, nb, sA, sB);
 }
 
 template<bool M3, bool FULL, int STAGE, int TAG>
@@ -691,3 +706,33 @@
     return ran;
 }
 void launch_gemm(const Launch& lc, const GemmArgs& a) { (void)launch_gemm_path(lc, a, -1); }
+
+int launch_gemm_pair(const Launch& lc, const GemmArgs& a0, const GemmArgs& a1) {
+    const GemmPlan p0 = gemm_plan(a0, lc.nb), p1 = gemm_plan(a1, lc.nb);
+    const int f0 = gemm_full_path(a0, p0), f1 = gemm_full_path(a1, p1);
+    const bool together = a0.tag == 1 && a1.tag == 1 && !a0.opA && !a1.opA && a0.M == a1.M && a0.N == a1.N && p0.tile == p1.tile &&
+                          p0.xcd == p1.xcd && p0.ksplit == 1 && p1.ksplit == 1 && f0 == f1 && f0 != 2;
+    if (!together) { launch_gemm(lc, a0); launch_gemm(lc, a1); return 2; }
+    const int t = ((a0.M + p0.tile - 1) / p0.tile) * ((a0.N + p0.tile - 1) / p0.tile);
+    const dim3 grid = p0.xcd ? dim3(t * lc.nb, 2, 1) : dim3(t, 2, lc.nb);
+    GemmPair pr;
+    pr.g[0] = a0; pr.g[1] = a1;
+    pr.g[0].ksplit = pr.g[1].ksplit = 1;
+    if (lc.sub) lc.sub->begin(lc.sub->user, SUBFAM_FACT_GEMM);
+    if (p0.tile == 64) {
+        if (f0) hipLaunchKernelGGL((k_zgemm_pair<2, 2, true, 1, 1>), grid, dim3(256), 0, lc.st, pr, lc.cs, lc.nb);
+        else    hipLaunchKernelGGL((k_zgemm_pair<2, 2, true, 1, 0>), grid, dim3(256), 0, lc.st, pr, lc.cs, lc.nb);
+    } else {
+        if (f0) hipLaunchKernelGGL((k_zgemm_pair<1, 1, true, 1, 1>), grid, dim3(256), 0, lc.st, pr, lc.cs, lc.nb);
+        else    hipLaunchKernelGGL((k_zgemm_pair<1, 1, true, 1, 0>), grid, dim3(256), 0, lc.st, pr, lc.cs, lc.nb);
+    }
+    if (lc.sub) {
+        double flops = 0.0, bytes = 0.0;
+        for (const GemmArgs* a : {&a0, &a1}) {
+            flops += 8.0 * a->M * a->N * a->K * lc.nb;
+            bytes += 16.0 * ((double)a->M * a->K + (double)a->K * a->N + (a->accumulate ? 2.0 : 1.0) * a->M * a->N) * lc.nb;
+        }
+        lc.sub->end(lc.sub->user, SUBFAM_FACT_GEMM, flops, bytes);
+    }
+    return 1;
+}
diff --git a/detqmc_amd/csrc/kernels_qr.hip b/detqmc_amd/csrc/kernels_qr.hip
--- a/detqmc_amd/csrc/kernels_qr.hip
+++ b/detqmc_amd/csrc/kernels_qr.hip
@@ -665,9 +665,14 @@
 }
 
 #define TRSM_NB 32
-__global__ __launch_bounds__(256) void k_trsm_block(cplx* __restrict__ C, int ldc, const cplx* __restrict__ R, int ldr,
-                                                     int n, int j0, int nb, int trans, int unit, size_t cs, ColSrc S) {
+struct TrsmPair { TrsmProblem p[2]; };
+__global__ __launch_bounds__(256) void k_trsm_block(TrsmPair pr, int ldc, const cplx* __restrict__ R, int ldr,
+                                                     int n, int j0, int nb, size_t cs) {
     __shared__ cplx sR[TRSM_NB][TRSM_NB + 1];
+    const TrsmProblem& P = pr.p[blockIdx.y ? 1 : 0];
+    cplx* __restrict__ C = P.C;
+    const int trans = P.trans, unit = P.unit;
+    ColSrc S = P.src;
     CHAIN(C); CHAIN(R); CHAIN(S.X); CHAIN(S.idx); CHAIN(S.scale);
     for (int i = threadIdx.x; i < TRSM_NB * TRSM_NB; i += 256) {
         int r = i % TRSM_NB, c = i / TRSM_NB;
@@ -727,29 +732,46 @@
     }
 }
 
-static int trsm_rec(const Launch& lc, int n, const cplx* R, cplx* C, int j0, int len, int trans, int unit, const ColSrc* src = nullptr) {
-    const ColSrc none = ColSrc();
+static int trsm_rec(const Launch& lc, int n, const cplx* R, const TrsmProblem* pb, int np, int j0, int len, bool first) {
     if (len <= TRSM_NB) {
-        hipLaunchKernelGGL(k_trsm_block, dim3((n + 255) / 256, 1, lc.nb), dim3(256), 0, lc.st, C, n, R, n, n, j0, len, trans, unit, lc.cs,
-                           src ? col_src_from(*src, j0) : none);
+        TrsmPair pr = TrsmPair();
+        for (int q = 0; q < np; ++q) {
+            pr.p[q] = pb[q];
+            pr.p[q].src = first ? col_src_from(pb[q].src, j0) : ColSrc();
+        }
+        hipLaunchKernelGGL(k_trsm_block, dim3((n + 255) / 256, np, lc.nb), dim3(256), 0, lc.st, pr, n, R, n, n, j0, len, lc.cs);
         return 1;
     }
     const int h = ((len / 2 + TRSM_NB - 1) / TRSM_NB) * TRSM_NB;
-    int launches = trsm_rec(lc, n, R, C, j0, h, trans, unit, src);
-    GemmArgs g = GemmArgs();
-    g.A = C + (size_t)j0 * n; g.lda = n; g.opA = 0; g.C = C + (size_t)(j0 + h) * n; g.ldc = n;
-    if (trans) { g.B = R + (size_t)j0 * n + (j0 + h); g.ldb = n; g.opB = 1; }
-    else       { g.B = R + (size_t)(j0 + h) * n + j0; g.ldb = n; g.opB = 0; }
-    g.M = n; g.N = len - h; g.K = h; g.Kmul = 1; g.accumulate = 1; g.negate = 1; g.tag = 1;
-    if (src) g.csrc = col_src_from(*src, j0 + h);
-    launch_gemm(lc, g);
-    launches += 1;
-    return launches + trsm_rec(lc, n, R, C, j0 + h, len - h, trans, unit);
+    int launches = trsm_rec(lc, n, R, pb, np, j0, h, first);
+    GemmArgs g[2];
+    for (int q = 0; q < np; ++q) {
+        cplx* C = pb[q].C;
+        g[q] = GemmArgs();
+        g[q].A = C + (size_t)j0 * n; g[q].lda = n; g[q].opA = 0; g[q].C = C + (size_t)(j0 + h) * n; g[q].ldc = n;
+        if (pb[q].trans) { g[q].B = R + (size_t)j0 * n + (j0 + h); g[q].ldb = n; g[q].opB = 1; }
+        else             { g[q].B = R + (size_t)(j0 + h) * n + j0; g[q].ldb = n; g[q].opB = 0; }
+        g[q].M = n; g[q].N = len - h; g[q].K = h; g[q].Kmul = 1; g[q].accumulate = 1; g[q].negate = 1; g[q].tag = 1;
+        if (first) g[q].csrc = col_src_from(pb[q].src, j0 + h);
+    }
+    if (np == 2) launches += launch_gemm_pair(lc, g[0], g[1]);
+    else { launch_gemm(lc, g[0]); launches += 1; }
+    return launches + trsm_rec(lc, n, R, pb, np, j0 + h, len - h, false);
+}
+static int trsm_rec(const Launch& lc, int n, const cplx* R, cplx* C, int j0, int len, int trans, int unit) {
+    const TrsmProblem p = {C, trans, unit, ColSrc()};
+    return trsm_rec(lc, n, R, &p, 1, j0, len, false);
 }
 int run_trsm_right_upper(const Launch& lc, int n, const cplx* R, cplx* C, const QrWork& w, int trans, int unit, const ColSrc* src) {
     (void)w;
-    if (src && (!src->X || src->X == C)) src = nullptr;
-    return trsm_rec(lc, n, R, C, 0, n, trans, unit, src);
+    TrsmProblem p = {C, trans, unit, ColSrc()};
+    if (src && src->X && src->X != C) p.src = *src;
+    return trsm_rec(lc, n, R, &p, 1, 0, n, true);
+}
+int run_trsm_right_upper_pair(const Launch& lc, int n, const cplx* R, const TrsmProblem& p0, const TrsmProblem& p1) {
+    TrsmProblem pb[2] = {p0, p1};
+    for (TrsmProblem& p : pb) if (p.src.X == p.C) p.src = ColSrc();
+    return trsm_rec(lc, n, R, pb, 2, 0, n, true);
 }
 
 #define BGS_NB 64
diff --git a/detqmc_amd/model.py b/detqmc_amd/model.py
--- a/detqmc_amd/model.py
+++ b/detqmc_amd/model.py
@@ -70,6 +70,7 @@
     decideThreads: int = 0
     bmultPath: int = 0
     rngLookahead: int = 0
+    trsmPair: int = 0
 
 
 OBSERVABLES = {"kOccX": 0, "kOccY": 1, "pairPlus": 2, "pairMinus": 3, "greenKTauX": 4, "greenKTauY": 5,
@@ -287,10 +288,14 @@
 ADAPT = {"box": 0, "rotate": 1, "scale": 2}
 
 
-def _tuning(pipeline=0, qrVariant=0, greenVariant=0, maxJacobiSweeps=0, proposalBudget=0, decideThreads=0, bmultPath=0, rngLookahead=0):
+def _tuning(pipeline=0, qrVariant=0, greenVariant=0, maxJacobiSweeps=0, proposalBudget=0, decideThreads=0, bmultPath=0, rngLookahead=0, trsmPair=0):
     if int(rngLookahead) not in (0, -1):
         raise ValueError("rngLookahead must be 0 (automatic: on) or -1 (off)")
-    path = int(bmultPath) | (_lib.DQMC_TUNING_NO_RNG_LOOKAHEAD if int(rngLookahead) == -1 and 0 <= int(bmultPath) <= 2 else 0)
+    if int(trsmPair) not in (0, -1):
+        raise ValueError("trsmPair must be 0 (automatic: paired on the LU route) or -1 (single solves)")
+    path = int(bmultPath)
+    if 0 <= path <= 2:
+        path |= (_lib.DQMC_TUNING_NO_RNG_LOOKAHEAD if int(rngLookahead) == -1 else 0) | (_lib.DQMC_TUNING_SINGLE_TRSM if int(trsmPair) == -1 else 0)
     return _lib.dqmc_tuning(pipeline=int(pipeline), qr_variant=int(qrVariant), green_variant=int(greenVariant),
                             max_jacobi_sweeps=int(maxJacobiSweeps), proposal_budget=int(proposalBudget),
                             decide_threads=int(decideThreads), bmult_path=path)
@@ -453,14 +458,14 @@
                  lambda_=1.0, txhor=-1.0, txver=-0.5, tyhor=0.5, tyver=1.0, mux=-0.5, muy=-0.5,
                  accRatio=0.5, phi2bosons=False, device=0, stabilisation="svd", checkerboard=True, nchains=1, cdwU=0.0,
                  pipeline=0, qrVariant=0, greenVariant=0, maxJacobiSweeps=0, proposalBudget=0, rngWindowPerSite=0, decideThreads=0, bmultPath=0,
-                 rngLookahead=0, timeDisplaced=False, tdParticleHole=False, tdCurrent=False, tdEverySlice=False, tdBand=False):
+                 rngLookahead=0, trsmPair=0, timeDisplaced=False, tdParticleHole=False, tdCurrent=False, tdEverySlice=False, tdBand=False):
         self.lib = load()
         p = _lib.dqmc_params(opdim=opdim, L=L, m=m, s=s, delaySteps=delaySteps, bc=BC[bc],
                              weakZflux=int(weakZflux), phi2bosons=int(phi2bosons), device=device,
                              stabilisation=STABILISATION[stabilisation], cb_none=int(not checkerboard), dtau=dtau, r=r, c=c, u=u, lambda_=lambda_, txhor=txhor, txver=txver,
                              tyhor=tyhor, tyver=tyver, mux=mux, muy=muy, accRatio=accRatio, cdwU=cdwU, rng_window_per_site=int(rngWindowPerSite),
                              timedisplaced=int(timeDisplaced) | (_lib.DQMC_TD_EVERY_SLICE if tdEverySlice else 0), td_particle_hole=(2 if tdCurrent else int(tdParticleHole)) | (_lib.DQMC_TD_PH_BAND if tdBand else 0),
-                             tuning=_tuning(pipeline, qrVariant, greenVariant, maxJacobiSweeps, proposalBudget, decideThreads, bmultPath, rngLookahead))
+                             tuning=_tuning(pipeline, qrVariant, greenVariant, maxJacobiSweeps, proposalBudget, decideThreads, bmultPath, rngLookahead, trsmPair))
         h = C.c_void_p()
         check(self.lib.dqmc_create_batch(C.byref(p), nchains, C.byref(h)))
         self.h = h
@@ -1095,7 +1100,7 @@
         | (_lib.DETSDW_TD_EVERY_SLICE if pars.timeDisplacedEverySlice else 0)
         | (_lib.DETSDW_TD_FINE_ON_DEVICE if pars.timeDisplacedFineOnDevice else 0),
         timeDisplacedParticleHole=(2 if pars.timeDisplacedCurrent else int(bool(pars.timeDisplacedParticleHole))) | (_lib.DETSDW_TD_PH_BAND if band_td else 0),
-        tuning=_tuning(pars.pipeline, pars.qrVariant, pars.greenVariant, pars.maxJacobiSweeps, pars.proposalBudget, pars.decideThreads, pars.bmultPath, pars.rngLookahead))
+        tuning=_tuning(pars.pipeline, pars.qrVariant, pars.greenVariant, pars.maxJacobiSweeps, pars.proposalBudget, pars.decideThreads, pars.bmultPath, pars.rngLookahead, pars.trsmPair))
 
 
 class DetSDW(_GreenCheck):
diff --git a/include/dqmc_hip.h b/include/dqmc_hip.h
--- a/include/dqmc_hip.h
+++ b/include/dqmc_hip.h
@@ -38,7 +38,8 @@
     int32_t decide_threads;
     int32_t bmult_path;
 } dqmc_tuning;
-enum { DQMC_TUNING_NO_RNG_LOOKAHEAD = 0x100 };
+enum { DQMC_TUNING_NO_RNG_LOOKAHEAD = 0x100, DQMC_TUNING_SINGLE_TRSM = 0x200 };
+enum { DQMC_TUNING_FLAG_BITS = DQMC_TUNING_NO_RNG_LOOKAHEAD | DQMC_TUNING_SINGLE_TRSM };
 
 typedef struct dqmc_params {
     int32_t opdim;
@@ -146,6 +147,9 @@
     uint64_t cholqr_fallbacks;
     uint64_t uniform_windows_advanced;
     uint64_t uniform_windows_pushed;
+    int32_t trsm_paired;
+    int32_t reserved0;
+    uint64_t trsm_pairs;
 } dqmc_schedule_info;
 int dqmc_get_schedule_info(dqmc_ctx* ctx, dqmc_schedule_info* out);
 int dqmc_get_update_state_host(dqmc_ctx* ctx, dqmc_update_state* out);
```

Result: no change. 299.5 sweeps/s (-0.1%).
